# ducha-aiki/mods-light-zmq

Measured on AMD Instinct MI355X. Metric: image_pairs_per_sec_end_to_end, higher is better.
Workload: dtype f32

## Files before the change

include/mods_hip.h:

```cpp
#ifndef MODS_HIP_H
#define MODS_HIP_H

#include <stddef.h>
#include <stdint.h>

#ifdef __cplusplus
extern "C" {
#endif

#define MODS_OK 0
#define MODS_E_NODEVICE (-1)
#define MODS_E_ARG (-2)
#define MODS_E_CAPACITY (-3)
#define MODS_E_HIP (-4)

typedef struct mods_ctx mods_ctx;

typedef struct mods_hessaff_params {
  int numberOfScales;
  float initialSigma;
  float threshold;
  float edgeEigenValueRatio;
  int border;
  int maxIterations;
  float convergenceThreshold;
  int smmWindowSize;
  int doBaumberg;
  int mode;
  float relativeThreshold;
  int regionsNumber;
  float relativeRegionsNumber;
  int detectorType;
  int iiDoGMode;
  int sampleFromImage;
  double mserMaxArea;
  double mserMinMargin;
  int mserMinSize;
  int affBmbrgMethod;
} mods_hessaff_params;
enum { MODS_DET_FIXED_TH = 0, MODS_DET_RELATIVE_TH, MODS_DET_FIXED_REG_NUMBER, MODS_DET_RELATIVE_REG_NUMBER,
       MODS_DET_NOT_LESS_THAN_REGIONS };
enum { MODS_DET_HESSIAN = 0, MODS_DET_DOG = 1, MODS_DET_HARRIS = 2, MODS_DET_MSER = 3 };

typedef struct mods_affkey {
  double x, y, s, a11, a12, a21, a22, response;
  int sub_type;
  int octave, level, r0, c0;
  int pad;
} mods_affkey;

typedef struct mods_candidate {
  int octave, level, r0, c0, r, c;
  float x, y, s, pixelDistance, response;
  int type;
} mods_candidate;

typedef struct mods_region {
  double x, y, s, a11, a12, a21, a22, response;
  int sub_type;
  int id, parent;
  int pad;
  uint8_t desc[128];
} mods_region;

typedef struct mods_tentative {
  int q, t;
  int t_bad, t_2nd;
  float d1, d2, d2nd;
  float pad;
  double ratio;
} mods_tentative;

const char *mods_last_error(void);
int mods_device_count(void);
int mods_ctx_create(int device, int max_w, int max_h, int batch, mods_ctx **out);
int mods_ctx_create_ex(int device, int max_w, int max_h, int batch, int flags, mods_ctx **out);
void mods_ctx_destroy(mods_ctx *ctx);
int mods_ctx_sync(mods_ctx *ctx);
void *mods_ctx_stream(mods_ctx *ctx);

enum { MODS_STAGE_BLUR = 0, MODS_STAGE_RESPONSE, MODS_STAGE_RESIZE, MODS_STAGE_NMS, MODS_STAGE_LOCALIZE,
       MODS_STAGE_BAUMBERG, MODS_STAGE_SORT, MODS_STAGE_ORIENT, MODS_STAGE_DESCRIBE, MODS_STAGE_MATCH,
       MODS_STAGE_RANSAC_SCORE, MODS_STAGE_SYNTH,
       MODS_STAGE_BLUR_SMALL,
       MODS_STAGE_PYRAMID,
       MODS_STAGE_MATCH_NN1,
       MODS_STAGE_EXTRACT,
       MODS_STAGE_SIFT,
       MODS_STAGE_GUIDED,
       MODS_STAGE_MATCH_MUTUAL,
       MODS_STAGE_OVERLAP,
       MODS_STAGE_COUNT };
int mods_ctx_timing_enable(mods_ctx *ctx, int stage_mask);
int mods_ctx_graphs(mods_ctx *ctx, int on);
long mods_ctx_graph_replays(const mods_ctx *ctx);
long mods_ctx_u8_source_calls(const mods_ctx *ctx);
int mods_ctx_u8_kernels(mods_ctx *ctx, int mask);
int mods_ctx_pyramid_streams(mods_ctx *ctx, int n);
int mods_ctx_timing_read(mods_ctx *ctx, int stage, double *total_ms, int *launches, double *bytes);
int mods_ctx_timing_reset(mods_ctx *ctx);

int mods_detect_hessian_affine(mods_ctx *ctx, const float *img, int w, int h, int stride,
                               const mods_hessaff_params *par, mods_affkey *out, int max_out, int *n_out);
int mods_detect_hessian_affine_dev(mods_ctx *ctx, const float *img_dev, int n_img, int w, int h, int stride,
                                   const mods_hessaff_params *par, mods_affkey *out_host, int max_out,
                                   int *n_out_host);

int mods_pyramid_octaves(mods_ctx *ctx);
int mods_pyramid_dims(mods_ctx *ctx, int octave, int *w, int *h);
int mods_pyramid_plane(mods_ctx *ctx, int img, int octave, int level, int kind, float *dst_host);
int mods_pyramid_candidates(mods_ctx *ctx, int img, mods_candidate *out, int max_out, int *n_out);
int mods_pyramid_nms_hits(mods_ctx *ctx, int img, int *out4, int max_out, int *n_out);

int mods_gauss_blur(mods_ctx *ctx, const float *src, int w, int h, float sigma, float *dst);
int mods_hessian_response(mods_ctx *ctx, const float *src, int w, int h, float norm, float *dst);
int mods_resize_half(mods_ctx *ctx, const float *src, int w, int h, float *dst, int *dw, int *dh);

typedef struct mods_describe_params {
  double ori_mrSize;
  int ori_patchSize;
  int ori_maxAngles;
  double ori_threshold;
  double desc_mrSize;
  int desc_patchSize;
  int photoNorm;
  int rootSift;
  double maxBinValue;
  int ori_halfMode;
  int addUpRight;
  int halfDesc;
  int fastExtraction;
} mods_describe_params;

int mods_orient_describe(mods_ctx *ctx, const float *img, int w, int h, int stride, const mods_affkey *keys,
                         int n_keys, const mods_describe_params *par, mods_region *out, int max_out, int *n_out);

int mods_orient_describe_u8(mods_ctx *ctx, const unsigned char *img_u8, int w, int h, int stride, const mods_affkey *keys,
                            int n_keys, const mods_describe_params *par, mods_region *out, int max_out, int *n_out);

int mods_detect_describe_dev(mods_ctx *ctx, const float *img_dev, int n_img, int w, int h, int stride,
                             const mods_hessaff_params *det, const mods_describe_params *desc,
                             int *n_detected_host, int *n_regions_host);
int mods_detect_describe_dev_u8(mods_ctx *ctx, const unsigned char *img_u8_dev, int n_img, int w, int h, int stride,
                                const mods_hessaff_params *det, const mods_describe_params *desc,
                                int *n_detected_host, int *n_regions_host);
typedef int (*mods_descriptor_fn)(void *user, const float *patches, int n, int ps, float *out, size_t out_cap_floats, int *dim);
int mods_ctx_set_external_descriptor(mods_ctx *ctx, mods_descriptor_fn fn, void *user, double mrSize, int patchSize);
int mods_ctx_set_external_shape(mods_ctx *ctx, mods_descriptor_fn fn, void *user, double mrSize, int patchSize);
int mods_ctx_set_external_orientation(mods_ctx *ctx, mods_descriptor_fn fn, void *user, double mrSize, int patchSize);
typedef struct mods_net mods_net;
enum { MODS_NET_AFFNET = 0, MODS_NET_ORINET = 1, MODS_NET_HARDNET = 2 };
int  mods_net_create(int device, int kind, const float *const *tensors, const size_t *n_floats, int n_tensors, mods_net **out);
void mods_net_destroy(mods_net *net);
int  mods_net_dim(const mods_net *net);
int  mods_net_chunk(void);
int  mods_net_forward(mods_net *net, const float *patches_host, int n, int quantise_u8, float *out_host);
int  mods_net_forward_dev(mods_net *net, void *hip_stream, const float *patches_dev, int n, int quantise_u8, float *out_dev);
int  mods_ctx_set_builtin_shape(mods_ctx *ctx, mods_net *net, double mrSize, int quantise_u8);
int  mods_ctx_set_builtin_orientation(mods_ctx *ctx, mods_net *net, double mrSize, int quantise_u8);
int  mods_ctx_set_builtin_descriptor(mods_ctx *ctx, mods_net *net, double mrSize, int quantise_u8);
int  mods_test_net_stage(mods_net *net, int stage, const float *in_host, int n, int quantise_u8, float *out_host, int *guard_ok);
int mods_patches_fetch(mods_ctx *ctx, int img, int ps, float *out, int max_regions, int *n_out);
int mods_baumberg_stats_enable(mods_ctx *ctx, int on);
int mods_baumberg_stats(mods_ctx *ctx, int img, unsigned long long *keypoints, unsigned long long *iterations);
int mods_unoriented_count(mods_ctx *ctx, int img);
int mods_regions_fetch(mods_ctx *ctx, int img, mods_region *out, int max_out, int *n_out);

int mods_dominant_angle(mods_ctx *ctx, const float *patch, int ps, double th, float *angle, int *found);
int mods_selftest_fast_sqrt(mods_ctx *ctx, unsigned long long *out5);
int mods_sift_patch(mods_ctx *ctx, const float *patch, int ps, int rootsift, double maxBinValue, uint8_t *out128);

typedef struct mods_view_geom {
  int identity;
  int w_rot, h_rot;
  int w_new, h_new;
  int ksize_x, ksize_y, pad;
  double rotation, tilt, zoom;
  double sigma_x, sigma_y;
  double H[9];
  double warpRot[6], warpTilt[6];
// ... 142 lines not shown
  int n_tentatives, n_unique, n_inliers;
  int ransac_samples, ransac_lo, ransac_rejects;
  double H[9];
  double ms_detect_describe, ms_match, ms_duplicates, ms_ransac;
  int gt_true, gt_ransac_inliers, gt_true_of_ransac;
} mods_ladder_result;

int mods_view_schedule(const double *scale_set, int n_scales, const double *tilt_set, int n_tilts, double phi_base,
                       mods_view_par *prev, int *n_prev, int prev_cap, mods_view_par *out, int max_out);
int mods_imgrep_create(mods_ctx *ctx, int capacity, mods_imgrep **out);
void mods_imgrep_destroy(mods_imgrep *rep);
int mods_imgrep_clear(mods_imgrep *rep);
int mods_imgrep_count(const mods_imgrep *rep);
const mods_region *mods_imgrep_regions_dev(const mods_imgrep *rep);
int mods_imgrep_append_ctx(mods_imgrep *rep, mods_ctx *ctx, int img);
int mods_imgrep_append_ctx_half(mods_imgrep *rep, mods_ctx *ctx, int img);
int mods_imgrep_append_dev(mods_imgrep *rep, const mods_region *src_dev, int n);
int mods_imgrep_append_host(mods_imgrep *rep, const mods_region *src, int n);
int mods_imgrep_fetch(mods_imgrep *rep, int begin, int count, mods_region *out);
int mods_match_reps(mods_ctx *ctx, const mods_imgrep *q, int q_begin, int q_end, const mods_imgrep *t, double ratio,
                    double contradDist, int nn, mods_tentative *out, double *u6_out, double *laf_out, int max_out, int *n_out);
int mods_match_ladder_dev(mods_ctx *ctx, const float *img1_dev, int w1, int h1, const float *img2_dev, int w2, int h2,
                          const mods_ladder_step *steps, int n_steps, int min_matches, const mods_pair_params *par,
                          mods_imgrep *rep1, mods_imgrep *rep2, mods_ladder_result *res, double *matches_out, int max_matches);

int mods_match_ladder_dets_dev(mods_ctx *ctx, const float *img1_dev, int w1, int h1, const float *img2_dev, int w2, int h2,
                               const mods_ladder_step *steps, const mods_hessaff_params *dets, int n_steps, int n_det, int min_matches,
                               const struct mods_pair_params *par, mods_imgrep **reps1, mods_imgrep **reps2, mods_ladder_result *res,
                               double *matches_out, int max_matches);

typedef struct mods_ladder_group {
  int n_dets, dets[8];
  double fginn_ratio, fginn_ratio_half;
  double dist_threshold, dist_threshold_half;
} mods_ladder_group;
int mods_match_ladder_groups_dev(mods_ctx *ctx, const float *img1_dev, int w1, int h1, const float *img2_dev, int w2, int h2,
                                 const mods_ladder_step *steps, const mods_hessaff_params *dets, const mods_ladder_group *groups ,
                                 int group_pos, int n_steps, int n_det, int min_matches, const struct mods_pair_params *par,
                                 mods_imgrep **reps1, mods_imgrep **reps2, mods_ladder_result *res, double *matches_out, int max_matches);

typedef struct mods_multi mods_multi;
int mods_multi_create(const int *devices, int n, int w, int h, int rep_capacity, mods_multi **out);
void mods_multi_destroy(mods_multi *m);
int mods_multi_uses_rccl(const mods_multi *m);
mods_imgrep *mods_multi_bank(mods_multi *m, int image);
mods_imgrep *mods_multi_bank_det(mods_multi *m, int image, int det);
int mods_match_ladder_multi(mods_multi *m, const float *img1_host, int w1, int h1, const float *img2_host, int w2, int h2,
                            const mods_ladder_step *steps, int n_steps, int min_matches, const mods_pair_params *par,
                            mods_ladder_result *res, double *matches_out, int max_matches);
int mods_match_ladder_groups_multi(mods_multi *m, const float *img1_host, int w1, int h1, const float *img2_host, int w2, int h2,
                                   const mods_ladder_step *steps, const mods_hessaff_params *dets, const mods_ladder_group *groups ,
                                   int group_pos, int n_steps, int n_det, int min_matches, const struct mods_pair_params *par,
                                   mods_ladder_result *res, double *matches_out, int max_matches);
int mods_match_reps_any(mods_ctx *ctx, const mods_imgrep *q, int q_begin, int q_end, const mods_imgrep *t, double ratio, double contradDist,
                        int nn, double distance, mods_tentative *out, double *u6_out, double *laf_out, int max_out, int *n_out);
int mods_regions_half_copy_dev(mods_ctx *ctx, int img, mods_region *dst_dev, int n);
int mods_multi_assign(const double *areas, int n, int n_dev, int *owner);

int mods_match_verify_reps(mods_ctx *ctx, mods_imgrep *rep1, mods_imgrep *rep2, double fginn_ratio, const mods_pair_params *par,
                           mods_ladder_result *res, double *matches_out, int max_matches);
int mods_host_alloc(size_t bytes, void **out);
int mods_host_free(void *p);
int mods_dev_alloc(size_t bytes, void **out);
int mods_dev_free(void *p);
int mods_dev_upload(void *dst_dev, const void *src_host, size_t bytes);
int mods_dev_download(void *dst_host, const void *src_dev, size_t bytes);

typedef struct mods_clahe_params { double clip_limit; int tiles_x, tiles_y; } mods_clahe_params;
int mods_clahe_dev(mods_ctx *ctx, const unsigned char *src_dev, int n_img, int w, int h, int src_stride,
                   const mods_clahe_params *par, void *dst_dev, int dst_stride, int dst_f32);
int mods_clahe(mods_ctx *ctx, const unsigned char *src_host, int w, int h, const mods_clahe_params *par, unsigned char *dst_host);

typedef struct mods_pipeline mods_pipeline;
int mods_pipeline_create(int device, int w, int h, const mods_pair_params *par, int gpu_workers, int verify_workers,
                         mods_pipeline **out);
int mods_pipeline_create_ex(int device, int w, int h, const mods_pair_params *par, int gpu_workers, int verify_workers,
                            int pairs_per_batch, mods_pipeline **out);
int mods_pipeline_create_clahe(int device, int w, int h, const mods_pair_params *par, int gpu_workers, int verify_workers,
                               int pairs_per_batch, const mods_clahe_params *clahe, mods_pipeline **out);
int mods_pipeline_capacity(const mods_pipeline *p);
int mods_pipeline_timing_enable(mods_pipeline *p, int stage_mask);
int mods_pipeline_timing_read(mods_pipeline *p, int stage, double *total_ms, int *launches, double *bytes);
long mods_pipeline_u8_source_calls(mods_pipeline *p);
long mods_pipeline_graph_replays(mods_pipeline *p);
int mods_pipeline_cpu_seconds(mods_pipeline *p, double *gpu_workers_s, double *verify_workers_s, int reset);
int mods_pipeline_submit(mods_pipeline *p, const float *img_dev, long tag);
int mods_pipeline_submit_host(mods_pipeline *p, const float *img_host, long tag);
int mods_pipeline_submit_host_u8(mods_pipeline *p, const unsigned char *img_host, long tag);
int mods_pipeline_next(mods_pipeline *p, mods_pair_result *res, long *tag);
int mods_pipeline_next_matches(mods_pipeline *p, mods_pair_result *res, long *tag, double *matches_out, int max_matches);
void mods_pipeline_destroy(mods_pipeline *p);

typedef struct mods_guided_params {
  int model_type;
  double model[9];
  double radius;
  double ratio;
  double contradDist;
  int max_dist;
  int one_to_one;
} mods_guided_params;
int mods_match_guided(mods_ctx *ctx, const mods_region *q, int n_q, const mods_region *t, int n_t,
                      const mods_guided_params *par, mods_tentative *out, double *u6_out, double *laf_out,
                      int max_out, int *n_out);
int mods_match_guided_reps(mods_ctx *ctx, const mods_imgrep *q, const mods_imgrep *t,
                           const mods_guided_params *par, mods_tentative *out, double *u6_out, double *laf_out,
                           int max_out, int *n_out);

typedef struct mods_overlap_params {
  double H[9];
  double max_error;
  int oriented;
  int one_to_one;
  int w1, h1, w2, h2;
} mods_overlap_params;
typedef struct mods_overlap_match { int q, t; double E, dist, diff; } mods_overlap_match;
typedef struct mods_overlap_counts { int n_q_common, n_t_common, n_matches; double repeatability; } mods_overlap_counts;
int mods_match_overlap(mods_ctx *ctx, const mods_region *q, int n_q, const mods_region *t, int n_t,
                       const mods_overlap_params *par, mods_overlap_match *out, int max_out, int *n_out,
                       mods_overlap_counts *counts);
int mods_match_overlap_reps(mods_ctx *ctx, const mods_imgrep *q, const mods_imgrep *t,
                            const mods_overlap_params *par, mods_overlap_match *out, int max_out, int *n_out,
                            mods_overlap_counts *counts);
int mods_ctx_overlap_splits(mods_ctx *ctx, int splits);

int mods_ctx_match_mutual(mods_ctx *ctx, int mode);
int mods_match_mutual_counts(mods_ctx *ctx, int *n_forward, int *n_kept);
int mods_pipeline_match_mutual(mods_pipeline *p, int mode);

#ifdef __cplusplus
}
#endif
#endif
```

mods-light-zmq_amd/__init__.py:

```python
import ctypes as C
import os
import subprocess

import numpy as np

PKG_DIR = os.path.dirname(os.path.abspath(__file__))
LIB_PATH = os.environ.get("MODS_LIB") or os.path.join(PKG_DIR, "libmodsgpu.so")

MODS_OK = 0
STAGES = ["blur", "response", "resize", "nms", "localize", "baumberg", "sort", "orient", "describe", "match",
          "ransac_score", "synth", "blur_small", "pyramid", "match_nn1", "extract", "sift", "guided", "match_mutual",
          "overlap"]


class ModsError(RuntimeError):
    pass


class HessAffParams(C.Structure):
    _fields_ = [("numberOfScales", C.c_int), ("initialSigma", C.c_float), ("threshold", C.c_float),
                ("edgeEigenValueRatio", C.c_float), ("border", C.c_int), ("maxIterations", C.c_int),
                ("convergenceThreshold", C.c_float), ("smmWindowSize", C.c_int), ("doBaumberg", C.c_int),
                ("mode", C.c_int), ("relativeThreshold", C.c_float), ("regionsNumber", C.c_int),
                ("relativeRegionsNumber", C.c_float), ("detectorType", C.c_int), ("iiDoGMode", C.c_int),
# ... 295 lines not shown
        params = params or HessAffParams.default()
        counts = (C.c_int * n_img)()
        out = np.zeros((n_img, max_out), AFFKEY_DTYPE) if fetch else None
        _check(lib().mods_detect_hessian_affine_dev(self.h, C.c_void_p(dev_ptr), n_img, w, h, w, C.byref(params),
                                                    out.ctypes.data_as(C.c_void_p) if fetch else None, max_out, counts))
        if fetch:
            return [out[i, :counts[i]].copy() for i in range(n_img)]
        return list(counts)

    def pyramid_octaves(self):
        return lib().mods_pyramid_octaves(self.h)

    def pyramid_dims(self, o):
        w, h = C.c_int(), C.c_int()
        _check(lib().mods_pyramid_dims(self.h, o, C.byref(w), C.byref(h)))
        return w.value, h.value

    def pyramid_plane(self, img, o, level, kind):
        w, h = self.pyramid_dims(o)
        out = np.empty((h, w), np.float32)
        _check(lib().mods_pyramid_plane(self.h, img, o, level, kind, _fp(out)))
        return out

    def pyramid_candidates(self, img=0, max_out=1 << 20):
        out = np.zeros(max_out, CAND_DTYPE)
        n = C.c_int()
        _check(lib().mods_pyramid_candidates(self.h, img, out.ctypes.data_as(C.c_void_p), max_out, C.byref(n)))
        return out[:n.value].copy()

    def pyramid_nms_hits(self, img=0, max_out=1 << 22):
        n = C.c_int()
        rc = lib().mods_pyramid_nms_hits(self.h, img, None, 0, C.byref(n))
        if rc not in (MODS_OK, -3):
            _check(rc)
        out = np.full((min(max(n.value, 0), max_out), 4), -1, np.int32)
        _check(lib().mods_pyramid_nms_hits(self.h, img, out.ctypes.data_as(C.c_void_p), len(out), C.byref(n)))
        return out[:int(np.count_nonzero(out[:, 1] >= 0))].copy(), n.value
    def orient_describe(self, img, keys, params=None, max_out=None):
        params = params or DescribeParams.default()
        a = np.ascontiguousarray(img, np.float32)
        k = np.ascontiguousarray(keys)
        max_out = max_out or len(k) + 1
        out = np.zeros(max_out, REGION_DTYPE)
        n = C.c_int()
        _check(lib().mods_orient_describe(self.h, _fp(a), a.shape[1], a.shape[0], a.shape[1], k.ctypes.data_as(C.c_void_p),
                                          len(k), C.byref(params), out.ctypes.data_as(C.c_void_p), max_out, C.byref(n)))
        return out[:n.value].copy()

    def orient_describe_u8(self, img_u8, keys, params=None, max_out=None):
        params = params or DescribeParams.default()
        a = np.asarray(img_u8)
        if a.dtype != np.uint8 or a.ndim != 2:
            raise ValueError("orient_describe_u8 takes a 2-d uint8 array")
        if a.strides[1] != 1 or a.strides[0] < a.shape[1]:
            a = np.ascontiguousarray(a)
        k = np.ascontiguousarray(keys)
        max_out = max_out or len(k) + 1
        out = np.zeros(max_out, REGION_DTYPE)
        n = C.c_int()
        _check(lib().mods_orient_describe_u8(self.h, C.c_void_p(a.ctypes.data), a.shape[1], a.shape[0], a.strides[0],
                                             k.ctypes.data_as(C.c_void_p), len(k), C.byref(params), out.ctypes.data_as(C.c_void_p),
                                             max_out, C.byref(n)))
        return out[:n.value].copy()

    def regions_fetch_half(self, img=0, max_out=1 << 18):
        out = np.zeros(max_out, REGION_DTYPE)
        n = C.c_int()
        _check(lib().mods_regions_fetch_half(self.h, img, out.ctypes.data_as(C.c_void_p), max_out, C.byref(n)))
        return out[:n.value].copy()

    def detect_describe_dev(self, dev_ptr, n_img, w, h, det=None, desc=None):
        det = det or HessAffParams.default()
        desc = desc or DescribeParams.default()
        nd, nr = (C.c_int * n_img)(), (C.c_int * n_img)()
        _check(lib().mods_detect_describe_dev(self.h, C.c_void_p(dev_ptr), n_img, w, h, w, C.byref(det), C.byref(desc), nd, nr))
        return list(nd), list(nr)

    def u8_source_calls(self):
        lib().mods_ctx_u8_source_calls.restype = C.c_long
        return int(lib().mods_ctx_u8_source_calls(self.h))

    def set_u8_kernels(self, mask):
        _check(lib().mods_ctx_u8_kernels(self.h, int(mask)))

    def set_match_mutual(self, mode):
        _check(lib().mods_ctx_match_mutual(self.h, int(mode)))

    def match_mutual_counts(self):
        nf, nk = C.c_int(), C.c_int()
        _check(lib().mods_match_mutual_counts(self.h, C.byref(nf), C.byref(nk)))
        return nf.value, nk.value

    def detect_describe_dev_u8(self, dev_ptr, n_img, w, h, det=None, desc=None, stride=None):
        det = det or HessAffParams.default()
        desc = desc or DescribeParams.default()
        nd, nr = (C.c_int * n_img)(), (C.c_int * n_img)()
        _check(lib().mods_detect_describe_dev_u8(self.h, C.c_void_p(dev_ptr), n_img, w, h, w if stride is None else int(stride),
                                                 C.byref(det), C.byref(desc), nd, nr))
        return list(nd), list(nr)

    def regions_fetch(self, img, max_out=1 << 18):
        n = C.c_int()
        _check(lib().mods_regions_fetch(self.h, img, None, 0, C.byref(n)))
        out = np.zeros(max(n.value, 1), REGION_DTYPE)
        _check(lib().mods_regions_fetch(self.h, img, out.ctypes.data_as(C.c_void_p), len(out), C.byref(n)))
        return out[:n.value].copy()

    def set_external_descriptor(self, fn_ptr, user, mr_size=3.0 * np.sqrt(3.0), patch_size=32):
        _check(lib().mods_ctx_set_external_descriptor(self.h, C.c_void_p(fn_ptr), C.c_void_p(user), C.c_double(mr_size), patch_size))

    def set_external_shape(self, fn_ptr, user, mr_size=3.0 * np.sqrt(3.0), patch_size=32):
        _check(lib().mods_ctx_set_external_shape(self.h, C.c_void_p(fn_ptr), C.c_void_p(user), C.c_double(mr_size), patch_size))

    def set_external_orientation(self, fn_ptr, user, mr_size=3.0 * np.sqrt(3.0), patch_size=32):
        _check(lib().mods_ctx_set_external_orientation(self.h, C.c_void_p(fn_ptr), C.c_void_p(user), C.c_double(mr_size), patch_size))

    def set_builtin_shape(self, net, mr_size=3.0 * np.sqrt(3.0), quantise=True):
        _slot_check("shape", net)
        _check(lib().mods_ctx_set_builtin_shape(self.h, net.h if net is not None else None, C.c_double(mr_size), 1 if quantise else 0))
        self._nets = dict(getattr(self, "_nets", {}), shape=net)

    def set_builtin_orientation(self, net, mr_size=3.0 * np.sqrt(3.0), quantise=True):
        _slot_check("orientation", net)
        _check(lib().mods_ctx_set_builtin_orientation(self.h, net.h if net is not None else None, C.c_double(mr_size), 1 if quantise else 0))
        self._nets = dict(getattr(self, "_nets", {}), orientation=net)

    def set_builtin_descriptor(self, net, mr_size=3.0 * np.sqrt(3.0), quantise=True):
        _slot_check("descriptor", net)
        _check(lib().mods_ctx_set_builtin_descriptor(self.h, net.h if net is not None else None, C.c_double(mr_size), 1 if quantise else 0))
        self._nets = dict(getattr(self, "_nets", {}), descriptor=net)

    def patches_fetch(self, img, ps, max_regions=1 << 17):
        n = C.c_int()
        out = np.zeros((max_regions, ps, ps), np.float32) if max_regions <= 4096 else None
        if out is None:
            cnt = C.c_int()
            _check(lib().mods_regions_fetch(self.h, img, None, 0, C.byref(cnt)))
            out = np.zeros((max(cnt.value, 1), ps, ps), np.float32)
        _check(lib().mods_patches_fetch(self.h, img, ps, _fp(out), out.shape[0], C.byref(n)))
        return out[:n.value].copy()

    def regions_copy_dev(self, img, dst_ptr, n):
        _check(lib().mods_regions_copy_dev(self.h, img, C.c_void_p(dst_ptr), n))

    def dominant_angle(self, patch, th=float(np.float32(0.8))):
        a = np.ascontiguousarray(patch, np.float32)
        ang, found = C.c_float(), C.c_int()
        _check(lib().mods_dominant_angle(self.h, _fp(a), a.shape[0], C.c_double(th), C.byref(ang), C.byref(found)))
        return bool(found.value), ang.value

    def selftest_fast_sqrt(self):
        out = (C.c_ulonglong * 5)()
        _check(lib().mods_selftest_fast_sqrt(self.h, out))
        return tuple(int(v) for v in out)

    def sift_patch(self, patch, rootsift=True, max_bin=0.2):
        a = np.ascontiguousarray(patch, np.float32)
        out = np.zeros(128, np.uint8)
        _check(lib().mods_sift_patch(self.h, _fp(a), a.shape[0], int(rootsift), C.c_double(max_bin),
                                     out.ctypes.data_as(C.c_void_p)))
        return out

    def warp_affine(self, img, M, dw, dh, cval=128.0):
        a = np.ascontiguousarray(img, np.float32)
        Mc = np.ascontiguousarray(M, np.float64).ravel()
        out = np.empty((dh, dw), np.float32)
# ... 605 lines not shown
def multi_assign(areas, n_dev):
    a = np.ascontiguousarray(areas, np.float64)
    owner = np.zeros(len(a), np.int32)
    _check(lib().mods_multi_assign(a.ctypes.data_as(C.c_void_p), len(a), n_dev, owner.ctypes.data_as(C.c_void_p)))
    return owner


def match_verify_reps(ctx, rep1, rep2, fginn_ratio=0.8, params=None, max_matches=0):
    params = params or PairParams.default()
    res = LadderResult()
    m = np.zeros((max(max_matches, 1), 4), np.float64)
    _check(lib().mods_match_verify_reps(ctx.h, rep1.h, rep2.h, C.c_double(fginn_ratio), C.byref(params), C.byref(res),
                                        m.ctypes.data_as(C.c_void_p) if max_matches else None, max_matches))
    return res, m[:min(res.n_inliers, max_matches)]


class PairParams(C.Structure):
    _fields_ = [("det", HessAffParams), ("desc", DescribeParams), ("fginn_ratio", C.c_double),
                ("contradDist", C.c_double), ("nn", C.c_int), ("dup_before_ransac", C.c_int),
                ("dup_dist", C.c_double), ("dup_mode", C.c_int), ("ransac", RansacParams)]

    @staticmethod
    def default():
        return PairParams(HessAffParams.default(), DescribeParams.default(), 0.8, 10.0, 50, 1, 2.0, 1,
                          RansacParams.default())


class PairResult(C.Structure):
    _fields_ = [("n_detected", C.c_int * 2), ("n_described", C.c_int * 2), ("n_tentatives", C.c_int),
                ("n_unique", C.c_int), ("n_inliers", C.c_int), ("ransac_samples", C.c_int), ("ransac_lo", C.c_int),
                ("ransac_rejects", C.c_int), ("H", C.c_double * 9), ("ms_detect_describe", C.c_double),
                ("ms_match", C.c_double), ("ms_duplicates", C.c_double), ("ms_ransac", C.c_double)]


def match_pair_dev(ctx, dev_ptr, w, h, params=None, max_matches=0):
    params = params or PairParams.default()
    res = PairResult()
    m = np.zeros((max(max_matches, 1), 4), np.float64)
    _check(lib().mods_match_pair_dev(ctx.h, C.c_void_p(dev_ptr), w, h, w, C.byref(params), C.byref(res),
                                     m.ctypes.data_as(C.c_void_p) if max_matches else None, max_matches))
    return res, m[:min(res.n_inliers, max_matches)]


class PinnedBuffer:

    def __init__(self, shape, dtype):
        self.shape, self.dtype = tuple(shape), np.dtype(dtype)
        self.nbytes = int(np.prod(self.shape)) * self.dtype.itemsize
        self.ptr = C.c_void_p()
        _check(lib().mods_host_alloc(C.c_size_t(self.nbytes), C.byref(self.ptr)))
        buf = (C.c_char * self.nbytes).from_address(self.ptr.value)
        self.array = np.frombuffer(buf, dtype=self.dtype).reshape(self.shape)

    def close(self):
        if self.ptr:
            self.array = None
            lib().mods_host_free(self.ptr)
            self.ptr = C.c_void_p()


class Pipeline:

    def __init__(self, device, w, h, params=None, gpu_workers=1, verify_workers=1, pairs_per_batch=1, clahe=None, mutual=0):
        self.params = params or PairParams.default()
        self.h = C.c_void_p()
        if clahe is not None:
            self.clahe = clahe
            _check(lib().mods_pipeline_create_clahe(device, w, h, C.byref(self.params), gpu_workers, verify_workers, pairs_per_batch,
                                                    C.byref(self.clahe), C.byref(self.h)))
        else:
            _check(lib().mods_pipeline_create_ex(device, w, h, C.byref(self.params), gpu_workers, verify_workers, pairs_per_batch,
                                                 C.byref(self.h)))
        self.capacity = lib().mods_pipeline_capacity(self.h)
        if mutual:
            try:
                self.set_match_mutual(mutual)
            except ModsError:
                self.close()
                raise

    def set_match_mutual(self, mode):
        _check(lib().mods_pipeline_match_mutual(self.h, int(mode)))

    def submit(self, dev_ptr, tag=0):
        _check(lib().mods_pipeline_submit(self.h, C.c_void_p(dev_ptr), C.c_long(tag)))

    def submit_host(self, host_ptr, tag=0, u8=False):
        fn = lib().mods_pipeline_submit_host_u8 if u8 else lib().mods_pipeline_submit_host
        _check(fn(self.h, C.c_void_p(host_ptr), C.c_long(tag)))

    def next(self):
        res, tag = PairResult(), C.c_long()
        _check(lib().mods_pipeline_next(self.h, C.byref(res), C.byref(tag)))
        return res, tag.value

    def next_matches(self, max_matches=1 << 16):
        res, tag = PairResult(), C.c_long()
        m = np.zeros((max_matches, 4), np.float64)
        _check(lib().mods_pipeline_next_matches(self.h, C.byref(res), C.byref(tag), m.ctypes.data_as(C.c_void_p), max_matches))
        return res, tag.value, m[:min(res.n_inliers, max_matches)]

    def timing_enable(self, stages):
        mask = 0
        for s in stages:
            mask |= 1 << STAGES.index(s)
        _check(lib().mods_pipeline_timing_enable(self.h, mask))

    def timing_read(self, stage):
        ms, n, by = C.c_double(), C.c_int(), C.c_double()
        _check(lib().mods_pipeline_timing_read(self.h, STAGES.index(stage), C.byref(ms), C.byref(n), C.byref(by)))
        return ms.value, n.value, by.value

    def graph_replays(self):
        lib().mods_pipeline_graph_replays.restype = C.c_long
        return int(lib().mods_pipeline_graph_replays(self.h))

    def u8_source_calls(self):
        lib().mods_pipeline_u8_source_calls.restype = C.c_long
        return int(lib().mods_pipeline_u8_source_calls(self.h))

    def cpu_seconds(self, reset=False):
        g, v = C.c_double(), C.c_double()
        _check(lib().mods_pipeline_cpu_seconds(self.h, C.byref(g), C.byref(v), 1 if reset else 0))
        return g.value, v.value

    def close(self):
        if self.h:
            lib().mods_pipeline_destroy(self.h)
            self.h = C.c_void_p()

    def __del__(self):
        try:
            self.close()
        except Exception:
            pass
```

mods-light-zmq_amd/csrc/capi.hip:

```cpp
#include "common.hpp"
#include "detmath.hpp"
#include "ransac_host.hpp"
#include "f_laf.hpp"
#include "../../include/mods_degensac.h"
#include <cstdarg>
#include <memory>
#include <algorithm>
#include <cmath>
#include <mutex>
#include <vector>
#include <time.h>
#include <sys/prctl.h>

namespace mods {

static thread_local char g_err[512] = "";

void set_error(const char *fmt, ...) {
  va_list ap;
  va_start(ap, fmt);
  vsnprintf(g_err, sizeof(g_err), fmt, ap);
  va_end(ap);
}

// ... 301 lines not shown
int mods_pyramid_plane(mods_ctx *c, int img, int o, int level, int kind, float *dst) {
  if (o < 0 || o >= c->pyr.n_oct || level < 0 || level >= c->pyr.n_levels || img < 0 || img >= c->last_n_img) return MODS_E_ARG;
  const OctaveDev &oc = c->pyr.oct[o];
  const float *p = (kind ? oc.resp[level] : oc.blur[level]) + (size_t)oc.w * oc.h * img;
  MODS_HIP_CHECK(mods::stream_wait(c->stream));
  MODS_HIP_CHECK(mods::copy_wait(c->stream, dst, p, sizeof(float) * (size_t)oc.w * oc.h, hipMemcpyDeviceToHost));
  return MODS_OK;
}
int mods_pyramid_candidates(mods_ctx *c, int img, mods_candidate *out, int max_out, int *n_out) {
  MODS_HIP_CHECK(mods::stream_wait(c->stream));
  int count = 0;
  MODS_HIP_CHECK(mods::copy_wait(c->stream, &count, c->cand_count + img, sizeof(int), hipMemcpyDeviceToHost));
  int n = std::min(count, c->max_cand);
  std::vector<CandDev> v(n);
  MODS_HIP_CHECK(mods::copy_wait(c->stream, v.data(), c->cand + (size_t)img * c->max_cand, sizeof(CandDev) * n, hipMemcpyDeviceToHost));
  int m = 0;
  for (auto &cd : v) {
    if (!(cd.state == 2 || cd.state == 3 || cd.state == 4)) continue;
    if (m < max_out) {
      mods_candidate &o = out[m];
      o.octave = cd.octave; o.level = cd.level; o.r0 = cd.r0; o.c0 = cd.c0; o.r = cd.r; o.c = cd.c;
      o.x = cd.x; o.y = cd.y; o.s = cd.s; o.pixelDistance = cd.pixelDistance; o.response = cd.response; o.type = cd.type;
    }
    m++;
  }
  *n_out = m;
  return m > max_out ? MODS_E_CAPACITY : MODS_OK;
}
int mods_pyramid_nms_hits(mods_ctx *c, int img, int *out4, int max_out, int *n_out) {
  if (!c || !n_out || img < 0 || img >= c->batch || (max_out > 0 && !out4)) { set_error("pyramid_nms_hits: bad argument"); return MODS_E_ARG; }
  MODS_HIP_CHECK(hipSetDevice(c->device));
  MODS_HIP_CHECK(mods::stream_wait(c->stream));
  int count = 0;
  MODS_HIP_CHECK(mods::copy_wait(c->stream, &count, c->cand_count + img, sizeof(int), hipMemcpyDeviceToHost));
  *n_out = count;
  const int n = std::max(0, std::min(count, c->max_cand));
  if (n > max_out) { set_error("NMS hit output overflow: %d > %d", n, max_out); return MODS_E_CAPACITY; }
  std::vector<CandDev> v(n);
  MODS_HIP_CHECK(mods::copy_wait(c->stream, v.data(), c->cand + (size_t)img * c->max_cand, sizeof(CandDev) * n, hipMemcpyDeviceToHost));
  for (int i = 0; i < n; i++) {
    out4[4 * i] = v[i].octave; out4[4 * i + 1] = v[i].level; out4[4 * i + 2] = v[i].r0; out4[4 * i + 3] = v[i].c0;
  }
  return MODS_OK;
}

static int check_desc_err(mods_ctx *c) {
  int e = 0;
  MODS_HIP_CHECK(hipMemcpyAsync(&e, c->desc_err_dev, sizeof(int), hipMemcpyDeviceToHost, c->stream));
  MODS_HIP_CHECK(mods::stream_wait(c->stream));
  if (e) {
    MODS_HIP_CHECK(hipMemsetAsync(c->desc_err_dev, 0, sizeof(int), c->stream));
    set_error("measurement region larger than the descriptor scratch (P2 > 3*max(w,h) or > 4096 blur taps)");
    return MODS_E_CAPACITY;
  }
  return MODS_OK;
}

static int dd_enqueue(mods_ctx *c, const float *img_dev, int n_img, int w, int h, int stride, const mods_hessaff_params *det,
                      const mods_describe_params *desc) {
  int rc;
  if ((rc = detect_any(c, img_dev, n_img, w, h, stride, det, 1.0, 1.0))) return rc;
  const float *planes = img_dev;
  if (stride != w) planes = c->tmp_dev;
  if ((rc = describe_run(c, planes, n_img, w, h, desc))) return rc;
  int *hc = c->host_counts;
  MODS_HIP_CHECK(hipMemcpyAsync(hc, c->cand_count, sizeof(int) * 3 * c->batch, hipMemcpyDeviceToHost, c->stream));
  MODS_HIP_CHECK(hipMemcpyAsync(hc + 3 * c->batch, c->region_count, sizeof(int) * c->batch, hipMemcpyDeviceToHost, c->stream));
  MODS_HIP_CHECK(hipMemcpyAsync(hc + 4 * c->batch, c->inside_count, sizeof(int) * n_img, hipMemcpyDeviceToHost, c->stream));
  MODS_HIP_CHECK(hipMemcpyAsync(hc + 5 * c->batch, c->desc_err_dev, sizeof(int), hipMemcpyDeviceToHost, c->stream));
  return MODS_OK;
}

static unsigned long long fnv1a(const void *p, size_t n, unsigned long long h) {
  const unsigned char *b = (const unsigned char *)p;
  for (size_t i = 0; i < n; i++) { h ^= b[i]; h *= 1099511628211ull; }
  return h;
}

static int dd_run(mods_ctx *c, const float *img_dev, int n_img, int w, int h, int stride, const mods_hessaff_params *det,
                  const mods_describe_params *desc) {
  const bool can = c->dd_graphs && c->timing_mask == 0 && !mods::has_hooks(c) && !mods::has_nets(c) && det->detectorType != MODS_DET_MSER;
  if (!can) { mods::dev_state_changed(c); return dd_enqueue(c, img_dev, n_img, w, h, stride, det, desc); }
  mods_ctx::DdKey key;
  key.img = img_dev; key.img_u8 = c->img_u8_dev; key.n_img = n_img; key.w = w; key.h = h; key.stride = stride;
  key.par_hash = fnv1a(desc, sizeof(*desc), fnv1a(det, sizeof(*det), 1469598103934665603ull)) ^ (unsigned long long)c->pyr_streams;
  key.epoch = c->dev_state_epoch;
  if (c->dd_stale) { dd_graph_drop(c); c->dd_linear.clear(); c->dd_stale = false; }
  const bool repeat = key == c->dd_prev;
  c->dd_prev = key;
  if (!repeat) return dd_enqueue(c, img_dev, n_img, w, h, stride, det, desc);
  for (auto &e : c->dd_cache)
    if (e.first == key) {
      MODS_HIP_CHECK(hipGraphLaunch(e.second, c->stream));
      c->dd_replays++;
      return MODS_OK;
    }
  for (const auto &k2 : c->dd_linear)
    if (k2 == key) return dd_enqueue(c, img_dev, n_img, w, h, stride, det, desc);
  hipStream_t s = c->stream;
  if (hipStreamBeginCapture(s, hipStreamCaptureModeThreadLocal) != hipSuccess) {
    (void)hipGetLastError();
    c->dd_graphs = false;
    return dd_enqueue(c, img_dev, n_img, w, h, stride, det, desc);
  }
  const int rc = dd_enqueue(c, img_dev, n_img, w, h, stride, det, desc);
  hipGraph_t g = nullptr;
  const hipError_t e_end = hipStreamEndCapture(s, &g);
  hipGraphExec_t ex = nullptr;
  if (rc == MODS_OK && e_end == hipSuccess && g && !c->pyr_forked) {
    (void)hipGraphDestroy(g);
    if (c->dd_linear.size() >= 16) c->dd_linear.erase(c->dd_linear.begin());
    c->dd_linear.push_back(key);
    return dd_enqueue(c, img_dev, n_img, w, h, stride, det, desc);
  }
  if (rc == MODS_OK && e_end == hipSuccess && g && hipGraphInstantiate(&ex, g, nullptr, nullptr, 0) == hipSuccess) {
    (void)hipGraphDestroy(g);
    if (c->dd_cache.size() >= 8) { (void)hipGraphExecDestroy(c->dd_cache.front().second); c->dd_cache.erase(c->dd_cache.begin()); }
    c->dd_cache.emplace_back(key, ex);
    MODS_HIP_CHECK(hipGraphLaunch(ex, c->stream));
    c->dd_replays++;
    return MODS_OK;
  }
  if (g) (void)hipGraphDestroy(g);
  (void)hipGetLastError();
  c->pyr_side = false;
  c->dd_graphs = false;
  c->omap_dirty = true;
  return dd_enqueue(c, img_dev, n_img, w, h, stride, det, desc);
}

int mods_ctx_graphs(mods_ctx *c, int on) {
  if (!c) return MODS_E_ARG;
  c->dd_graphs = on != 0;
  if (!on) { dd_graph_drop(c); c->dd_linear.clear(); }
  mods::dev_state_changed(c);
  return MODS_OK;
}
long mods_ctx_graph_replays(const mods_ctx *c) { return c ? c->dd_replays : 0; }
long mods_ctx_u8_source_calls(const mods_ctx *c) { return c ? c->u8_source_calls : 0; }
int mods_ctx_u8_kernels(mods_ctx *c, int mask) {
  if (!c || mask > 15) { set_error("u8_kernels: bad argument"); return MODS_E_ARG; }
  c->u8_kernels = mask < 0 ? -1 : mask;
  mods::dev_state_changed(c);
  return MODS_OK;
}

static int dd_call(mods_ctx *c, const float *img_dev, int n_img, int w, int h, int stride, const mods_hessaff_params *det,
                   const mods_describe_params *desc, int *n_detected_host, int *n_regions_host) {
  int rc;
  if ((rc = dd_run(c, img_dev, n_img, w, h, stride, det, desc))) return rc;
  int *hc = c->host_counts;
  MODS_HIP_CHECK(mods::stream_wait(c->stream));
  for (int b = 0; b < n_img; b++) {
    if (hc[b] > c->max_cand) { set_error("NMS hit list overflow: %d > %d", hc[b], c->max_cand); return MODS_E_CAPACITY; }
    if (n_detected_host) n_detected_host[b] = hc[2 * c->batch + b];
    if (hc[3 * c->batch + b] > std::min(c->max_cand, 1 << 17)) { set_error("region list overflow: %d", hc[3 * c->batch + b]); return MODS_E_CAPACITY; }
    if (n_regions_host) n_regions_host[b] = hc[3 * c->batch + b];
  }
  c->last_region_counts.assign(hc + 3 * c->batch, hc + 3 * c->batch + n_img);
  c->last_inside_counts.assign(hc + 4 * c->batch, hc + 4 * c->batch + n_img);
  if (hc[5 * c->batch]) {
    MODS_HIP_CHECK(hipMemsetAsync(c->desc_err_dev, 0, sizeof(int), c->stream));
    set_error("measurement region larger than the descriptor scratch (P2 > 3*max(w,h) or > 4096 blur taps)");
    return MODS_E_CAPACITY;
  }
  return MODS_OK;
}

int mods_detect_describe_dev(mods_ctx *c, const float *img_dev, int n_img, int w, int h, int stride,
                             const mods_hessaff_params *det, const mods_describe_params *desc, int *n_detected_host,
                             int *n_regions_host) {
  if (!c || !img_dev || !det || !desc) { set_error("detect_describe: null argument"); return MODS_E_ARG; }
  if (w <= 0 || h <= 0 || (size_t)w * h > (size_t)c->max_w * c->max_h) { set_error("detect_describe: image larger than the context"); return MODS_E_ARG; }
  if (n_img < 1 || n_img > c->batch) { set_error("detect_describe: %d images, context batch %d", n_img, c->batch); return MODS_E_ARG; }
  if (stride < w) { set_error("detect_describe: stride %d < width %d", stride, w); return MODS_E_ARG; }
  MODS_HIP_CHECK(hipSetDevice(c->device));
  c->img_u8_dev = nullptr;
  return dd_call(c, img_dev, n_img, w, h, stride, det, desc, n_detected_host, n_regions_host);
}

int mods_detect_describe_dev_u8(mods_ctx *c, const unsigned char *img_u8_dev, int n_img, int w, int h, int stride,
                                const mods_hessaff_params *det, const mods_describe_params *desc, int *n_detected_host,
                                int *n_regions_host) {
  if (!c || !img_u8_dev || !det || !desc) { set_error("detect_describe_u8: null argument"); return MODS_E_ARG; }
  if (w <= 0 || h <= 0 || (size_t)w * h > (size_t)c->max_w * c->max_h) { set_error("detect_describe_u8: image larger than the context"); return MODS_E_ARG; }
  if (n_img < 1 || n_img > c->batch) { set_error("detect_describe_u8: %d images, context batch %d", n_img, c->batch); return MODS_E_ARG; }
  if (stride < w) { set_error("detect_describe_u8: stride %d < width %d", stride, w); return MODS_E_ARG; }
  MODS_HIP_CHECK(hipSetDevice(c->device));
  int rc;
  if ((rc = mods::u8_to_f32_launch(c, img_u8_dev, n_img, w, h, stride, c->input_dev))) return rc;
  c->img_u8_dev = (stride == w && det->detectorType != MODS_DET_MSER) ? img_u8_dev : nullptr;
  if (c->img_u8_dev) c->u8_source_calls++;
  rc = dd_call(c, c->input_dev, n_img, w, h, w, det, desc, n_detected_host, n_regions_host);
  c->img_u8_dev = nullptr;
  return rc;
}

int mods_ctx_set_external_descriptor(mods_ctx *c, mods_descriptor_fn fn, void *user, double mrSize, int patchSize) {
  if (!c) return MODS_E_ARG;
  c->ext_fn = fn; c->ext_user = user; c->ext_mr = mrSize; c->ext_ps = patchSize;
  c->ext_net = nullptr;
  return MODS_OK;
}

int mods_ctx_set_external_shape(mods_ctx *c, mods_descriptor_fn fn, void *user, double mrSize, int patchSize) {
  if (!c) return MODS_E_ARG;
  if (fn && (patchSize < 8 || patchSize > 63)) { set_error("external shape: patch size %d unsupported", patchSize); return MODS_E_ARG; }
  c->shape_fn = fn; c->shape_user = user; c->shape_mr = mrSize; c->shape_ps = patchSize;
  c->shape_net = nullptr;
  return MODS_OK;
}

int mods_ctx_set_external_orientation(mods_ctx *c, mods_descriptor_fn fn, void *user, double mrSize, int patchSize) {
  if (!c) return MODS_E_ARG;
  if (fn && (patchSize < 8 || patchSize > 63)) { set_error("external orientation: patch size %d unsupported", patchSize); return MODS_E_ARG; }
  c->ori_fn = fn; c->ori_user = user; c->ori_mr = mrSize; c->ori_ps = patchSize;
  c->ori_net = nullptr;
  return MODS_OK;
}
int mods_patches_fetch(mods_ctx *c, int img, int ps, float *out, int max_regions, int *n_out) {
  if (!c || !out || !n_out || img < 0 || img >= c->batch || !c->desc_scratch) { set_error("patches_fetch: nothing described"); return MODS_E_ARG; }
  const int reg_cap = std::min(c->max_cand, 1 << 17);
  MODS_HIP_CHECK(hipSetDevice(c->device));
  MODS_HIP_CHECK(mods::stream_wait(c->stream));
  int n = 0;
  MODS_HIP_CHECK(mods::copy_wait(c->stream, &n, c->region_count + img, sizeof(int), hipMemcpyDeviceToHost));
  if (n > reg_cap) n = reg_cap;
  if (n > max_regions) { set_error("patch output overflow: %d > %d", n, max_regions); return MODS_E_CAPACITY; }
  MODS_HIP_CHECK(mods::copy_wait(c->stream, out, c->desc_scratch + (size_t)img * reg_cap * ps * ps, sizeof(float) * (size_t)n * ps * ps, hipMemcpyDeviceToHost));
  *n_out = n;
  return MODS_OK;
}

int mods_baumberg_stats_enable(mods_ctx *c, int on) {
  if (!c) return MODS_E_ARG;
  MODS_HIP_CHECK(hipSetDevice(c->device));
  MODS_HIP_CHECK(mods::stream_wait(c->stream));
  c->baum_stats_dev.release();
  mods::dev_pool_reallocated(c);
  if (on) {
    const size_t n = 2 * 64 * (size_t)c->batch;
    MODS_HIP_CHECK(c->baum_stats_dev.reserve(n));
    MODS_HIP_CHECK(mods::fill_wait(c->stream, c->baum_stats_dev, 0, sizeof(unsigned long long) * n));
  }
  return MODS_OK;
}
int mods_baumberg_stats(mods_ctx *c, int img, unsigned long long *keypoints, unsigned long long *iterations) {
  if (!c || img < 0 || img >= c->batch || !c->baum_stats_dev) return MODS_E_ARG;
  MODS_HIP_CHECK(hipSetDevice(c->device));
  MODS_HIP_CHECK(mods::stream_wait(c->stream));
  unsigned long long v[2 * 64], kp = 0, it = 0;
  MODS_HIP_CHECK(mods::copy_wait(c->stream, v, c->baum_stats_dev + 2 * 64 * (size_t)img, sizeof(v), hipMemcpyDeviceToHost));
  for (int q = 0; q < 64; q++) { kp += v[2 * q]; it += v[2 * q + 1]; }
  if (keypoints) *keypoints = kp;
  if (iterations) *iterations = it;
  return MODS_OK;
}

int mods_unoriented_count(mods_ctx *c, int img) {
  if (!c || img < 0 || img >= (int)c->last_inside_counts.size()) return 0;
  return c->last_inside_counts[img];
}

int mods_regions_fetch(mods_ctx *c, int img, mods_region *out, int max_out, int *n_out) {
  if (!c || img < 0 || img >= c->batch || !n_out) return MODS_E_ARG;
  MODS_HIP_CHECK(hipSetDevice(c->device));
  MODS_HIP_CHECK(mods::stream_wait(c->stream));
  int n = 0;
  MODS_HIP_CHECK(mods::copy_wait(c->stream, &n, c->region_count + img, sizeof(int), hipMemcpyDeviceToHost));
  *n_out = n;
  if (out) {
    if (n > max_out) { set_error("region output overflow: %d > %d", n, max_out); return MODS_E_CAPACITY; }
    MODS_HIP_CHECK(mods::copy_wait(c->stream, out, c->regions_dev + (size_t)img * c->max_cand, sizeof(mods_region) * n, hipMemcpyDeviceToHost));
  }
  return MODS_OK;
}

int mods_regions_fetch_half(mods_ctx *c, int img, mods_region *out, int max_out, int *n_out) {
  if (!c || img < 0 || img >= c->batch || !n_out) return MODS_E_ARG;
  if (!c->have_half || !c->regions_half_dev) { set_error("no HalfRootSIFT descriptors: the last describe call did not ask for them"); return MODS_E_ARG; }
  MODS_HIP_CHECK(hipSetDevice(c->device));
  MODS_HIP_CHECK(mods::stream_wait(c->stream));
  int n = 0;
  MODS_HIP_CHECK(mods::copy_wait(c->stream, &n, c->region_count + img, sizeof(int), hipMemcpyDeviceToHost));
  *n_out = n;
  if (out) {
    if (n > max_out) { set_error("region output overflow: %d > %d", n, max_out); return MODS_E_CAPACITY; }
    MODS_HIP_CHECK(mods::copy_wait(c->stream, out, c->regions_half_dev + (size_t)img * c->max_cand, sizeof(mods_region) * n, hipMemcpyDeviceToHost));
  }
  return MODS_OK;
}
const mods_region *mods_regions_half_dev(mods_ctx *c, int img) {
  return (c && c->have_half && c->regions_half_dev) ? c->regions_half_dev + (size_t)img * c->max_cand : nullptr;
}

int mods_orient_describe(mods_ctx *c, const float *img, int w, int h, int stride, const mods_affkey *keys, int n_keys,
                         const mods_describe_params *par, mods_region *out, int max_out, int *n_out) {
  if (!c || !img || !par || !n_out || (n_keys > 0 && !keys)) { set_error("orient_describe: null argument"); return MODS_E_ARG; }
  if ((size_t)w * h > (size_t)c->max_w * c->max_h) { set_error("image larger than the context"); return MODS_E_ARG; }
  if (n_keys > c->max_cand) { set_error("too many keypoints for the context: %d > %d", n_keys, c->max_cand); return MODS_E_CAPACITY; }
  MODS_HIP_CHECK(hipSetDevice(c->device));
  MODS_HIP_CHECK(hipMemcpy2DAsync(c->input_dev, sizeof(float) * w, img, sizeof(float) * stride, sizeof(float) * w, h,
                                  hipMemcpyHostToDevice, c->stream));
  MODS_HIP_CHECK(hipMemcpyAsync(c->keys_dev, keys, sizeof(mods_affkey) * n_keys, hipMemcpyHostToDevice, c->stream));
  MODS_HIP_CHECK(hipMemcpyAsync(c->cand_count + 2 * c->batch, &n_keys, sizeof(int), hipMemcpyHostToDevice, c->stream));
  MODS_HIP_CHECK(mods::stream_wait(c->stream));
  int rc = describe_run(c, c->input_dev, 1, w, h, par);
  if (rc) return rc;
  if ((rc = mods_regions_fetch(c, 0, out, max_out, n_out))) return rc;
  return check_desc_err(c);
}

int mods_orient_describe_u8(mods_ctx *c, const unsigned char *img_u8, int w, int h, int stride, const mods_affkey *keys, int n_keys,
                            const mods_describe_params *par, mods_region *out, int max_out, int *n_out) {
  if (!img_u8 || !par || !n_out || (n_keys > 0 && !keys)) { set_error("orient_describe_u8: null argument"); return MODS_E_ARG; }
  if (w < 1 || h < 1) { set_error("orient_describe_u8: image size %d x %d", w, h); return MODS_E_ARG; }
  if (stride < w) { set_error("orient_describe_u8: stride %d < width %d", stride, w); return MODS_E_ARG; }
  if (n_keys < 0) { set_error("orient_describe_u8: %d keypoints", n_keys); return MODS_E_ARG; }
  if (!c) { set_error("orient_describe_u8: null context"); return MODS_E_ARG; }
  if ((size_t)w * h > (size_t)c->max_w * c->max_h) { set_error("orient_describe_u8: image %d x %d larger than the context", w, h); return MODS_E_ARG; }
  if (n_keys > c->max_cand) { set_error("orient_describe_u8: too many keypoints for the context: %d > %d", n_keys, c->max_cand); return MODS_E_ARG; }
  MODS_HIP_CHECK(hipSetDevice(c->device));
  int rc;
  if ((rc = mods::u8_stage_ensure(c))) return rc;
  MODS_HIP_CHECK(hipMemcpy2DAsync(c->u8_stage_dev, w, img_u8, stride, w, h, hipMemcpyHostToDevice, c->stream));
  MODS_HIP_CHECK(hipMemcpyAsync(c->keys_dev, keys, sizeof(mods_affkey) * n_keys, hipMemcpyHostToDevice, c->stream));
  MODS_HIP_CHECK(hipMemcpyAsync(c->cand_count + 2 * c->batch, &n_keys, sizeof(int), hipMemcpyHostToDevice, c->stream));
  MODS_HIP_CHECK(mods::stream_wait(c->stream));
  if ((rc = mods::u8_to_f32_launch(c, c->u8_stage_dev, 1, w, h, w, c->input_dev))) return rc;
  c->img_u8_dev = c->u8_stage_dev;
  c->u8_source_calls++;
  rc = describe_run(c, c->input_dev, 1, w, h, par);
  c->img_u8_dev = nullptr;
  if (rc) return rc;
  if ((rc = mods_regions_fetch(c, 0, out, max_out, n_out))) return rc;
  return check_desc_err(c);
}

int mods_dominant_angle(mods_ctx *c, const float *patch, int ps, double th, float *angle, int *found) {
  mods_describe_params dp = {5.1962, ps, 1, th, 5.1962, c->desc_ps ? c->desc_ps : 41, 1, 1, 0.2};
  MODS_HIP_CHECK(hipSetDevice(c->device));
  int rc = describe_configure(c, &dp);
  if (rc) return rc;
  MODS_HIP_CHECK(hipMemcpyAsync(c->input_dev, patch, sizeof(float) * ps * ps, hipMemcpyHostToDevice, c->stream));
  if ((rc = launch_dominant_angle_test(c, c->input_dev, ps, th, c->tmp_dev))) return rc;
  float res[2];
  MODS_HIP_CHECK(hipMemcpyAsync(res, c->tmp_dev, sizeof(res), hipMemcpyDeviceToHost, c->stream));
  MODS_HIP_CHECK(mods::stream_wait(c->stream));
  *found = res[0] != 0.f;
  *angle = res[1];
  return MODS_OK;
}

int mods_selftest_fast_sqrt(mods_ctx *c, unsigned long long *out5) {
  if (!c || !out5) { set_error("selftest: null argument"); return MODS_E_ARG; }
  MODS_HIP_CHECK(hipSetDevice(c->device));
  return launch_fast_sqrt_selftest(c, out5);
}

int mods_sift_patch(mods_ctx *c, const float *patch, int ps, int rootsift, double maxBinValue, uint8_t *out128) {
  mods_describe_params dp = {5.1962, c->desc_ori_ps ? c->desc_ori_ps : 32, 1, 0.8, 5.1962, ps, 1, rootsift, maxBinValue};
  MODS_HIP_CHECK(hipSetDevice(c->device));
  int rc = describe_configure(c, &dp);
  if (rc) return rc;
  MODS_HIP_CHECK(hipMemcpyAsync(c->input_dev, patch, sizeof(float) * ps * ps, hipMemcpyHostToDevice, c->stream));
  if ((rc = launch_sift_patch_test(c, c->input_dev, ps, rootsift, maxBinValue, (uint8_t *)c->tmp_dev.get()))) return rc;
  MODS_HIP_CHECK(hipMemcpyAsync(out128, c->tmp_dev, 128, hipMemcpyDeviceToHost, c->stream));
  MODS_HIP_CHECK(mods::stream_wait(c->stream));
  return MODS_OK;
}

int mods_match_copy_out(mods_ctx *c, int n, mods_tentative *tent, double *u6, double *laf) {
  if (n <= 0) return MODS_OK;
  static thread_local std::vector<char> stage;
  stage.resize(tent_bytes((size_t)n));
  MODS_HIP_CHECK(hipMemcpyAsync(stage.data(), c->m_tent, stage.size(), hipMemcpyDeviceToHost, c->stream));
  MODS_HIP_CHECK(mods::stream_wait(c->stream));
  tent_unpack(stage.data(), (size_t)n, tent, u6, laf);
  return MODS_OK;
}

int mods_match_fetch_internal(mods_ctx *c, mods_tentative *out, double *u6_out, double *laf_out, int max_out, int *n_out) {
  MODS_HIP_CHECK(mods::stream_wait(c->stream));
  const int n = read_slot(c->m_count, count_slot());
  *n_out = n;
  if (n > max_out) { set_error("tentative output overflow: %d > %d", n, max_out); return MODS_E_CAPACITY; }
  return mods_match_copy_out(c, n, out, u6_out, laf_out);
}

static int match_upload(mods_ctx *c, const mods_region *q, int n_q, const mods_region *t, int n_t, const int *n_out) {
  if (!c || !n_out || (n_q > 0 && !q) || (n_t > 0 && !t)) { set_error("match: null argument"); return MODS_E_ARG; }
  MODS_HIP_CHECK(hipSetDevice(c->device));
  int rc = match_ensure_buffers(c);
  if (rc) return rc;
  if (n_q > c->max_cand || n_t > c->max_cand) { set_error("match: list larger than the context capacity"); return MODS_E_CAPACITY; }
  MODS_HIP_CHECK(hipMemcpyAsync(c->m_regs, q, sizeof(mods_region) * n_q, hipMemcpyHostToDevice, c->stream));
  MODS_HIP_CHECK(hipMemcpyAsync(c->m_regs + c->max_cand, t, sizeof(mods_region) * n_t, hipMemcpyHostToDevice, c->stream));
  return MODS_OK;
}

int mods_match_fginn(mods_ctx *c, const mods_region *q, int n_q, const mods_region *t, int n_t, double ratio,
                     double contradDist, int nn, mods_tentative *out, double *u6_out, double *laf_out, int max_out, int *n_out) {
  int rc = match_upload(c, q, n_q, t, n_t, n_out);
  if (rc || (rc = match_run(c, c->m_regs, n_q, c->m_regs + c->max_cand, n_t, ratio, contradDist, nn))) return rc;
  return mods_match_fetch_internal(c, out, u6_out, laf_out, max_out, n_out);
}

int mods_match_distance(mods_ctx *c, const mods_region *q, int n_q, const mods_region *t, int n_t, double threshold,
                        mods_tentative *out, double *u6_out, double *laf_out, int max_out, int *n_out) {
  int rc = match_upload(c, q, n_q, t, n_t, n_out);
  if (rc || (rc = match_run_distance(c, c->m_regs, n_q, c->m_regs + c->max_cand, n_t, threshold))) return rc;
  return mods_match_fetch_internal(c, out, u6_out, laf_out, max_out, n_out);
}

int mods_match_dev(mods_ctx *c, int img_q, int img_t, double ratio, double contradDist, int nn, mods_tentative *out,
                   double *u6_out, double *laf_out, int max_out, int *n_out) {
// ... 379 lines not shown
```

mods-light-zmq_amd/csrc/common.hpp:

```cpp
#pragma once
#include <hip/hip_runtime.h>
#include <atomic>
#include <chrono>
#include <cmath>
#include <cstdint>
#include <cstdio>
#include <cstring>
#include <string>
#include <vector>
#include "../../include/mods_hip.h"
#include "buffer.hpp"

namespace mods {

void set_error(const char *fmt, ...);

#define MODS_HIP_CHECK(expr)                                                              \
  do {                                                                                    \
    hipError_t _e = (expr);                                                               \
    if (_e != hipSuccess) {                                                               \
      mods::set_error("%s failed: %s (%s:%d)", #expr, hipGetErrorString(_e), __FILE__, __LINE__); \
      return MODS_E_HIP;                                                                  \
    }                                                                                     \
  } while (0)
// ... 87 lines not shown
}

struct TentList {
  std::vector<mods_tentative> tent;
  std::vector<double> u6, laf;
  size_t size() const { return tent.size(); }
  bool empty() const { return tent.empty(); }
  void clear() { tent.clear(); u6.clear(); laf.clear(); }
  void resize(size_t n) { tent.resize(n); u6.resize(n * 6); laf.resize(n * 14); }
  void truncate(size_t n) { if (n < size()) resize(n); }
  void append(const TentList &o) {
    tent.insert(tent.end(), o.tent.begin(), o.tent.end());
    u6.insert(u6.end(), o.u6.begin(), o.u6.end());
    laf.insert(laf.end(), o.laf.begin(), o.laf.end());
  }
  void unpack_from(const char *packed, size_t n) { resize(n); tent_unpack(packed, n, tent.data(), u6.data(), laf.data()); }
  void pack_into(char *packed) const { tent_pack(packed, size(), tent.data(), u6.data(), laf.data()); }
  void copy_matches(int n, double *matches_out, int max_matches) const {
    if (!matches_out) return;
    for (int m = 0; m < n && m < max_matches && (size_t)m < size(); m++) {
      const double *p = &u6[(size_t)m * 6];
      matches_out[4 * m] = p[0]; matches_out[4 * m + 1] = p[1]; matches_out[4 * m + 2] = p[3]; matches_out[4 * m + 3] = p[4];
    }
  }
};

constexpr int kCountSlots = 64;
constexpr int kCountInts = 3 * kCountSlots;
constexpr int kLastSearch = -1;
constexpr int count_slot(int pair = kLastSearch) { return 1 + pair; }
constexpr int kept_slot(int pair = kLastSearch) { return kCountSlots + 1 + pair; }
constexpr int status_slot(int pair = kLastSearch) { return 2 * kCountSlots + 1 + pair; }
inline int read_slot(const int *counts, int slot) { return ((const volatile int *)counts)[slot]; }

struct MserState;

}

struct mods_ctx {
  mods_ctx() = default;
  ~mods_ctx();
  int device = 0;
  int n_cu = 256;
  int max_w = 0, max_h = 0, batch = 1;
  hipStream_t stream = nullptr;
  hipEvent_t pyr_scope_begin = nullptr;
  hipStream_t stream2 = nullptr;
  hipEvent_t ev_fork = nullptr, ev_join = nullptr;
  bool pyr_side = false;
  int pyr_side_first = 0;
  int pyr_streams = 2;
  mods::PyramidDev pyr;
  mods::Buf<mods::PyramidDev> pyr_dev;
  mods::PyramidDev pyr_dev_image;
  bool pyr_dev_valid = false;
  mods::Buf<float> plane_pool;
  mods::Buf<unsigned int> omap_pool;
  bool omap_dirty = true;
  mods::Buf<float> input_dev;
  mods::Buf<float> tmp_dev;
  mods::Buf<float> alt_taps_dev;
  int alt_ntap[mods::kMaxLevels] = {0};
  float alt_sigma[mods::kMaxLevels] = {0};
  mods::Buf<float> alt_planes;
  mods::Buf<float> view_dev;
  mods::Buf<float> gauss_taps_dev;
  float taps_sigma[16] = {0};
  float taps_host[16][2 * mods::kMaxBlurRadius + 1] = {{0}};
  int taps_host_n[16] = {0};
  mods::Buf<float> smm_mask_dev;
  mods::Buf<unsigned long long> baum_stats_dev;
  int smm_mask_size = 0;
  int max_cand = 0;
  mods::Buf<mods::CandDev> cand;
  mods::Buf<int> cand_count;
  mods::Buf<mods_affkey> keys_dev;
  mods::Buf<unsigned long long> sort_keys;
  mods::Buf<int> sort_idx;
  mods::Buf<int> rank_dev;
  mods::Buf<unsigned long long> nms_mask;
  mods::PinnedBuf<int> host_counts;
  mods::Buf<unsigned char> u8_stage_dev;
  const unsigned char *img_u8_dev = nullptr;
  int u8_kernels = -1;
  long u8_source_calls = 0;
  mods::Buf<unsigned char> clahe_lut;
  bool clahe_on = false;
  mods_clahe_params clahe_par = {0.0, 0, 0};
  mods::PinnedBuf<char> pin_arena;
  mods_hessaff_params par;
  int reg_number_eff = -1;
  int last_w = 0, last_h = 0, last_n_img = 0;
  const float *last_img_dev = nullptr; int last_stride = 0;
  mods::Buf<float> desc_tables_dev;
  mods::Buf<int> desc_err_dev;
  int desc_ori_ps = 0, desc_ps = 0;
  mods::Buf<char> ori_dev;
  mods::Buf<char> ori_multi_dev;
  mods::Buf<mods_region> regions_dev;
  mods::Buf<mods_region> regions_half_dev;
  bool have_half = false;
  mods::Buf<int> region_count;
  mods::Buf<int> inside_count;
  std::vector<int> last_inside_counts;
  mods::Buf<float> desc_scratch;
  int blur_table_ps = 0;
  mods::Buf<float> blur_table_dev;
  mods_descriptor_fn ext_fn = nullptr;
  void *ext_user = nullptr;
  double ext_mr = 0;
  int ext_ps = 0;
  mods_descriptor_fn shape_fn = nullptr, ori_fn = nullptr;
  void *shape_user = nullptr, *ori_user = nullptr;
  double shape_mr = 0, ori_mr = 0;
  int shape_ps = 0, ori_ps = 0;
  mods_net *shape_net = nullptr, *ori_net = nullptr, *ext_net = nullptr;
  int shape_q8 = 0, ori_q8 = 0, ext_q8 = 0;
  mods::Buf<float> net_out_dev;
  std::vector<int> last_region_counts;
  mods::Buf<int8_t> m_desc;
  mods::Buf<int> m_c;
  mods::Buf<double2> m_xy;
  mods::Buf<unsigned long long> m_u64;
  mods::Buf<int> m_int;
  mods::Buf<char> m_mid;
  mods::Buf<char> m_p2;
  size_t m_best2_cap = 0;
  int m_sets = 0;
  mods::Buf<char> m_tent;
  mods::PinnedBuf<int> m_count;
  mods_tentative *m_tent_out = nullptr; int *m_count_out = nullptr;
  mods::Buf<char> m_tent_batch;
  mods::Buf<mods_region> m_regs;
  mods::Buf<char> dd_buf; int dd_jobs = 0;
  mods::Buf<char> m_tent2;
  mods::TentList h_list;
  std::vector<unsigned char> h_mask;
  mods::Buf<double4> g_rec;
  mods::Buf<unsigned char> g_desc;
  mods::Buf<unsigned long long> g_key;
  mods::Buf<int> g_int;
  mods::Buf<char> g_tent;
  mods::Buf<mods_region> g_regs;
  mods::PinnedBuf<int> g_count;
  mods::Buf<double> o_rec;
  mods::Buf<unsigned long long> o_key;
  mods::Buf<int> o_int;
  mods::Buf<mods_overlap_match> o_out;
  mods::Buf<mods_region> o_regs;
  mods::PinnedBuf<int> o_count;
  int o_splits = 0;
  int mutual_mode = 0;
  bool mu_last_checked = false;
  mods::Buf<int4> mu_cand;
  mods::PinnedBuf<int> mu_count;
  mods::MserState *mser = nullptr;
  std::vector<mods_ctx *> helpers;
  std::atomic<bool> helpers_failed{false};
  std::vector<mods::Buf<mods_region>> helper_stage;
  int timing_mask = 0;
  bool dd_graphs = false;
  struct DdKey { const float *img = nullptr; const unsigned char *img_u8 = nullptr;
                 int n_img = 0, w = 0, h = 0, stride = 0; unsigned long long par_hash = 0, epoch = ~0ull;
                 bool operator==(const DdKey &o) const { return img == o.img && img_u8 == o.img_u8 && n_img == o.n_img && w == o.w && h == o.h && stride == o.stride && par_hash == o.par_hash && epoch == o.epoch; } };
  unsigned long long dev_state_epoch = 0;
  std::vector<std::pair<DdKey, hipGraphExec_t>> dd_cache;
  bool dd_stale = false;
  DdKey dd_prev;
  std::vector<DdKey> dd_linear;
  bool pyr_forked = false;
  long dd_replays = 0;
  mods::StageTimer timers[MODS_STAGE_COUNT];
};

namespace mods {

constexpr int kTabOriMask = 0, kTabDescMask = 4096, kTabVoteMask = 8192, kTabSift = 12288;

inline void dev_state_changed(mods_ctx *c) { c->dev_state_epoch++; }
inline void dev_pool_reallocated(mods_ctx *c) { c->dev_state_epoch++; c->dd_stale = true; }

template <class B> inline hipError_t reserve_scratch(mods_ctx *c, B &b, size_t need, size_t alloc_elems, bool *moved = nullptr) {
  if (need <= b.capacity()) return hipSuccess;
  if (b.get()) { const hipError_t e = stream_wait(c->stream); if (e != hipSuccess) return e; }
  return b.reserve(need, alloc_elems, moved);
}
template <class B> inline hipError_t reserve_pool(mods_ctx *c, B &b, size_t need, size_t alloc_elems) {
  bool moved = false;
  const hipError_t e = reserve_scratch(c, b, need, alloc_elems, &moved);
  if (moved) dev_pool_reallocated(c);
  return e;
}
struct StageScope {
  mods_ctx *ctx; int stage; hipEvent_t e0 = nullptr, e1 = nullptr; bool on;
  StageScope(mods_ctx *c, int s, double bytes = 0);
  ~StageScope();
};

int pyramid_configure(mods_ctx *ctx, int w, int h, int n_img, const mods_hessaff_params *par);
int pyramid_build(mods_ctx *ctx, const float *img_dev, int stride);
int pyramid_join_side(mods_ctx *ctx);
int launch_gauss_blur(mods_ctx *ctx, const float *src, float *dst, int w, int h, int n_img, float sigma);
int launch_hessian_response(mods_ctx *ctx, const float *src, float *dst, int w, int h, int n_img, float norm);
int launch_resize_half(mods_ctx *ctx, const float *src, float *dst, int w, int h, int dw, int dh, int n_img);
void resize_half_dims(int w, int h, int *dw, int *dh);
int gauss_ksize(float sigma);
void gauss_kernel_host(int n, double sigma, float *out);
void gauss_mask_host(int size, float *out);
void circular_gauss_mask_host(int size, float sigma, float *out);

int clahe_reserve(mods_ctx *ctx, int n_img, const mods_clahe_params *par);
int clahe_launch(mods_ctx *ctx, const unsigned char *src, int n_img, int w, int h, int src_stride, const mods_clahe_params *par,
                 void *dst, int dst_stride, int dst_f32);

int detect_run(mods_ctx *ctx);

int detect_any(mods_ctx *ctx, const float *img_dev, int n_img, int w, int h, int stride, const mods_hessaff_params *par, double tilt,
               double zoom);
void mser_release(mods_ctx *ctx);

int match_run(mods_ctx *ctx, const mods_region *q_dev, int n_q, const mods_region *t_dev, int n_t, double ratio,
              double contradDist, int nn);
int match_run_distance(mods_ctx *ctx, const mods_region *q_dev, int n_q, const mods_region *t_dev, int n_t, double threshold);
int match_ensure_buffers(mods_ctx *ctx, int n_sets = 1);
int match_run_group(mods_ctx *ctx, int n_jobs, const mods_region *const *q_dev, const int *n_q, const mods_region *const *t_dev, const int *n_t,
                    mods_tentative *const *tent_out, int *const *count_out, double ratio, double contradDist, int nn);

constexpr int DUP_MAX_JOBS = 64;
struct DupJob { const char *src; char *dst; const int *n_src; int *n_dst; int *status; };
int dup_filter_dev(mods_ctx *c, const DupJob *jobs, int n_jobs, int grid_n, double r, int mode);
int dup_filter_reserve(mods_ctx *c, int n_jobs);
static_assert(DUP_MAX_JOBS <= kCountSlots, "every job of the duplicate filter has its slots in m_count");
int launch_fast_sqrt_selftest(mods_ctx *ctx, unsigned long long *out5_host);
int launch_blur_table(mods_ctx *ctx, int ps);
bool ransac_profile_on();
int ransac_profile_mode();

int describe_run(mods_ctx *ctx, const float *img_dev, int n_img, int w, int h, const mods_describe_params *par);
int u8_to_f32_launch(mods_ctx *c, const unsigned char *src, int n_img, int w, int h, int stride, float *dst);
int u8_stage_ensure(mods_ctx *c);
int describe_run_view(mods_ctx *ctx, const float *img_dev, int n_img, int w, int h, const mods_describe_params *par, const double *H,
                      int orig_w, int orig_h, mods_region *det_copy_dev);
int describe_configure(mods_ctx *ctx, const mods_describe_params *par);
int launch_dominant_angle_test(mods_ctx *ctx, const float *patch_dev, int ps, double th, float *out_dev);
int launch_sift_patch_test(mods_ctx *ctx, const float *patch_dev, int ps, int root, double max_bin, uint8_t *out_dev);

inline bool has_hooks(const mods_ctx *c) { return c->ext_fn || c->shape_fn || c->ori_fn; }
inline bool has_nets(const mods_ctx *c) { return c->ext_net || c->shape_net || c->ori_net; }
int net_run_to_host(mods_ctx *ctx, mods_net *net, const float *patches_dev, int n, int quantise_u8, float *out_host);

int pair_gpu_stage(mods_ctx *c, const float *img_dev, int w, int h, int stride, const mods_pair_params *par, mods_pair_result *res,
                   TentList *list);
int pairs_gpu_stage(mods_ctx *c, const void *const *img, const int *kinds, int n_pairs, int w, int h, const mods_pair_params *par,
                    mods_pair_result *const *res, TentList *const *lists);
int pair_verify_stage(int device, const mods_pair_params *par, mods_pair_result *res, TentList *list, double *matches_out,
                      int max_matches, int w, int h);

}

extern "C" {
int mods_match_copy_out(mods_ctx *c, int n, mods_tentative *tent, double *u6, double *laf);
int mods_match_fetch_internal(mods_ctx *c, mods_tentative *out, double *u6_out, double *laf_out, int max_out, int *n_out);
int mods_ransac_warmup(int device, int len);
int mods_ctx_warmup(mods_ctx *c, int n_img, int w, int h, const mods_pair_params *par);
}
```

mods-light-zmq_amd/csrc/describe.hip:

```cpp
#include "describe_common.hpp"
#include "detmath.hpp"
#include "device_util.hpp"

namespace mods {

struct OriOut { double a11, a12, a21, a22; int alive; int pad; };

__device__ unsigned char g_ori_bin[2048];
__global__ __launch_bounds__(256) void ori_bin_table_kernel() {
  const float PIf = 3.14159265358979323846f;
  const int bins = 36;
  const int e = blockIdx.x * 256 + threadIdx.x;
  const float ori = atan2_lut_case(e >> 8, g_atan_lut[e & 255]);
  g_ori_bin[e] = (unsigned char)(int)(bins * (ori / PIf + 1.0f) / 2.0f);
}

__device__ __forceinline__ float peak_angle(const float *s_hist, int b) {
  const int bins = 36;
  const float PIf = 3.14159265358979323846f;
  const int a = b == 0 ? bins - 1 : b - 1, c = b == bins - 1 ? 0 : b + 1;
  const float ha = s_hist[a], hb = s_hist[b], hc = s_hist[c];
  const float pp = (ha - hc) / (ha - 2.0f * hb + hc) / 2.0f;
  return 2.0f * PIf * (b + 0.5f + pp) / bins - PIf;
}
// ... 612 lines not shown
      if (ctx->ori_net) {
        if ((rc = net_run_to_host(ctx, ctx->ori_net, ctx->desc_scratch + (size_t)b * k.reg_cap * kNetPS * kNetPS, n, ctx->ori_q8, out.data()))) return rc;
      } else {
        int dim = 0;
        const int frc = ctx->ori_fn(ctx->ori_user, patches[b].data(), n, ctx->ori_ps, out.data(), out.size(), &dim);
        if (frc || dim != 2) { set_error("external orientation function failed (rc %d, %d values per patch; 2 expected)", frc, dim); return MODS_E_ARG; }
      }
      for (int i = 0; i < n; i++) {
        mods_region r = regs[b][i];
        const double angle = atan2f(out[2 * i], out[2 * i + 1]);
        double ci, si;
        det_sincos(angle, &si, &ci);
        const double a11 = r.a11, a12 = r.a12, a21 = r.a21, a22 = r.a22;
        r.a11 = a11 * ci - a12 * si;
        r.a12 = a11 * si + a12 * ci;
        r.a21 = a21 * ci - a22 * si;
        r.a22 = a21 * si + a22 * ci;
        const int box = (int)(k.ks * r.s);
        bool alive = true;
        if (k.view) {
          const double rx = (k.Hinv[0] * r.x + k.Hinv[1] * r.y + k.Hinv[2]);
          const double ry = (k.Hinv[3] * r.x + k.Hinv[4] * r.y + k.Hinv[5]);
          const double r11 = (k.Hinv[0] * r.a11 + k.Hinv[1] * r.a21), r12 = (k.Hinv[0] * r.a12 + k.Hinv[1] * r.a22);
          const double r21 = (k.Hinv[3] * r.a11 + k.Hinv[4] * r.a21), r22 = (k.Hinv[3] * r.a12 + k.Hinv[4] * r.a22);
          if (!((rx < k.ow) && (ry < k.oh) && (rx > 0) && (ry > 0))) alive = false;
          else if (check_borders(k.ow, k.oh, (float)rx, (float)ry, (float)r11, (float)r12, (float)r21, (float)r22, box, box)) alive = false;
        } else if (check_borders(k.w, k.h, (float)r.x, (float)r.y, (float)r.a11, (float)r.a12, (float)r.a21, (float)r.a22, box, box)) alive = false;
        if (!alive) continue;
        r.parent = r.id; r.id = (int)kept.size();
        kept.push_back(r);
      }
    }
    counts[b] = (int)kept.size();
    if (counts[b] > k.reg_cap) counts[b] = k.reg_cap;
    if (counts[b]) MODS_HIP_CHECK(mods::copy_wait(ctx->stream, ctx->regions_dev + (size_t)b * ctx->max_cand, kept.data(), sizeof(mods_region) * counts[b], hipMemcpyHostToDevice));
  }
  MODS_HIP_CHECK(mods::copy_wait(ctx->stream, ctx->region_count, counts.data(), sizeof(int) * n_img, hipMemcpyHostToDevice));
  MODS_HIP_CHECK(mods::copy_wait(ctx->stream, ctx->inside_count, inside.data(), sizeof(int) * n_img, hipMemcpyHostToDevice));
  return MODS_OK;
}

static void invert3_cv(const double *S, double *t) {
  double d = S[0] * (S[4] * S[8] - S[5] * S[7]) - S[1] * (S[3] * S[8] - S[5] * S[6]) + S[2] * (S[3] * S[7] - S[4] * S[6]);
  if (d == 0.) { for (int i = 0; i < 9; i++) t[i] = 0; return; }
  d = 1. / d;
  t[0] = (S[4] * S[8] - S[5] * S[7]) * d; t[1] = (S[2] * S[7] - S[1] * S[8]) * d; t[2] = (S[1] * S[5] - S[2] * S[4]) * d;
  t[3] = (S[5] * S[6] - S[3] * S[8]) * d; t[4] = (S[0] * S[8] - S[2] * S[6]) * d; t[5] = (S[2] * S[3] - S[0] * S[5]) * d;
  t[6] = (S[3] * S[7] - S[4] * S[6]) * d; t[7] = (S[1] * S[6] - S[0] * S[7]) * d; t[8] = (S[0] * S[4] - S[1] * S[3]) * d;
}

int describe_run_view(mods_ctx *ctx, const float *img_dev, int n_img, int w, int h, const mods_describe_params *par, const double *H,
                      int orig_w, int orig_h, mods_region *det_copy_dev) {
  int rc = describe_configure(ctx, par);
  if (rc) return rc;
  DescConst k;
  k.view = 0; k.ow = w; k.oh = h;
  for (int i = 0; i < 6; i++) k.Hinv[i] = (i == 0 || i == 4) ? 1.0 : 0.0;
  if (H) {
    const bool eye = (std::fabs(H[0] - 1.0) + std::fabs(H[1]) + std::fabs(H[2]) + std::fabs(H[3]) + std::fabs(H[4] - 1.0) + std::fabs(H[5]) +
                      std::fabs(H[6]) + std::fabs(H[7]) + std::fabs(H[8] - 1.0) < 0.01);
    k.ow = orig_w; k.oh = orig_h;
    if (!eye) {
      double Hi[9];
      invert3_cv(H, Hi);
      k.view = 1;
      for (int i = 0; i < 6; i++) k.Hinv[i] = Hi[i];
    } else if (orig_w != w || orig_h != h) k.view = 1;
  }
  k.w = w; k.h = h; k.max_cand = ctx->max_cand; k.max_reg = ctx->max_cand;
  k.reg_cap = std::min(ctx->max_cand, 1 << 17);
  k.ks = 2 * 3.0 * sqrt(3.0);
  k.ori_ps = par->ori_patchSize;
  k.ori_i2p = double(2 * int(par->ori_mrSize) + 1) / (double)par->ori_patchSize;
  k.max_angles = par->ori_maxAngles;
  k.ori_cap = std::max(1, std::min(par->ori_maxAngles, 18));
  k.ori_th = par->ori_threshold;
  k.ori_half = par->ori_halfMode; k.half_desc = 0; k.add_upright = par->addUpRight;
  k.desc_mr = par->desc_mrSize; k.desc_ps = par->desc_patchSize; k.photo = par->photoNorm; k.root = par->rootSift;
  k.max_bin = par->maxBinValue;
  k.patch_rule = par->fastExtraction ? 2 : 0;
  const bool external = ctx->ext_fn != nullptr || ctx->ext_net != nullptr;
  const bool hooks = external || ctx->shape_fn || ctx->shape_net || ctx->ori_fn || ctx->ori_net;
  const unsigned char *img_u8 = (!H && !hooks) ? ctx->img_u8_dev : nullptr;
  if (external && par->fastExtraction) { set_error("FastPatchExtraction with an external descriptor is not supported"); return MODS_E_ARG; }
  if (external) { k.desc_mr = ctx->ext_mr; k.desc_ps = ctx->ext_ps; k.photo = 0; k.patch_rule = 1; }
  int *key_count = ctx->cand_count + 2 * ctx->batch;
  const float *orimask = ctx->desc_tables_dev + kTabVoteMask, *dmask = ctx->desc_tables_dev + kTabDescMask;
  const SiftTab *tab = (const SiftTab *)(ctx->desc_tables_dev + kTabSift);
  if ((ctx->shape_fn || ctx->shape_net) && ctx->par.detectorType == MODS_DET_HESSIAN && (rc = external_shape(ctx, img_dev, n_img, k, key_count, dmask, tab))) return rc;
  if (ctx->ori_fn || ctx->ori_net) {
    if ((rc = external_orientation(ctx, img_dev, n_img, k, key_count, dmask, tab))) return rc;
  } else {
    StageScope ts(ctx, MODS_STAGE_ORIENT);
    const size_t lds = orient_lds_bytes(k.ori_ps);
    hipLaunchKernelGGL(ori_bin_table_kernel, dim3(8), dim3(256), 0, ctx->stream);
    if (k.ori_cap > 1) {
      const size_t need = sizeof(OriOut) * (size_t)k.ori_cap * ctx->max_cand * ctx->batch;
      MODS_HIP_CHECK(mods::reserve_pool(ctx, ctx->ori_multi_dev, need, need));
    }
    if (img_u8 && kernel_from_u8(ctx, U8K_ORIENT))
      hipLaunchKernelGGL(orient_kernel<unsigned char>, dim3(8192, n_img), dim3(64), lds, ctx->stream, img_u8, k, ctx->keys_dev, key_count,
                         orimask, (OriOut *)ctx->ori_dev.get(), (OriOut *)ctx->ori_multi_dev.get());
    else
      hipLaunchKernelGGL(orient_kernel<float>, dim3(8192, n_img), dim3(64), lds, ctx->stream, img_dev, k, ctx->keys_dev, key_count,
                         orimask, (OriOut *)ctx->ori_dev.get(), (OriOut *)ctx->ori_multi_dev.get());
    if (k.ori_cap > 1)
      hipLaunchKernelGGL(compact_regions_multi_kernel, dim3(1, n_img), dim3(1024), 0, ctx->stream, k, ctx->keys_dev, key_count,
                         (const OriOut *)ctx->ori_dev.get(), (const OriOut *)ctx->ori_multi_dev.get(), ctx->regions_dev, ctx->region_count, ctx->inside_count);
    else
      hipLaunchKernelGGL(compact_regions_kernel, dim3((ctx->max_cand + 1023) / 1024, n_img), dim3(1024), 0, ctx->stream, k, ctx->keys_dev, key_count,
                         (const OriOut *)ctx->ori_dev.get(), ctx->regions_dev, ctx->region_count, ctx->inside_count);
    MODS_HIP_CHECK(hipGetLastError());
  }
  rc = launch_extract_and_sift(ctx, img_dev, n_img, k, dmask, tab, !external, img_u8);
  if (rc) return rc;
  ctx->have_half = false;
  if (par->halfDesc && !external) {
    if ((rc = launch_half_sift(ctx, n_img, k, dmask, tab))) return rc;
    ctx->have_half = true;
  }
  if (external && (rc = external_describe(ctx, n_img, k))) return rc;
  if (det_copy_dev)
    MODS_HIP_CHECK(hipMemcpyAsync(det_copy_dev, ctx->regions_dev, sizeof(mods_region) * (size_t)ctx->max_cand, hipMemcpyDeviceToDevice, ctx->stream));
  if (k.view) {
    hipLaunchKernelGGL(reproject_regions_kernel, dim3(256, n_img), dim3(256), 0, ctx->stream, k, ctx->regions_dev, ctx->region_count);
    if (ctx->have_half)
      hipLaunchKernelGGL(reproject_regions_kernel, dim3(256, n_img), dim3(256), 0, ctx->stream, k, ctx->regions_half_dev, ctx->region_count);
    MODS_HIP_CHECK(hipGetLastError());
  }
  return MODS_OK;
}

int launch_dominant_angle_test(mods_ctx *ctx, const float *patch_dev, int ps, double th, float *out_dev) {
  const size_t lds = orient_lds_bytes(ps);
  hipLaunchKernelGGL(ori_bin_table_kernel, dim3(8), dim3(256), 0, ctx->stream);
  hipLaunchKernelGGL(dominant_angle_test_kernel, dim3(1), dim3(64), lds, ctx->stream, patch_dev, ps, th,
                     ctx->desc_tables_dev + kTabVoteMask, out_dev);
  MODS_HIP_CHECK(hipGetLastError());
  return MODS_OK;
}

}
```

mods-light-zmq_amd/csrc/describe_common.hpp:

```cpp
#pragma once
#include "common.hpp"

namespace mods {

struct DescConst {
  int w, h;
  int max_cand, max_reg;
  int reg_cap;
  double ks;
  int ori_ps;
  double ori_i2p;
  int max_angles;
  int ori_cap;
  double ori_th;
  int ori_half;
  int add_upright;
  int half_desc;
  double desc_mr;
  int desc_ps;
  int photo, root;
  double max_bin;
  int p2_lo, p2_hi;
  size_t scratch_stride;
  int tap_cap;
  int patch_rule;
  int view;
  int ow, oh;
  double Hinv[6];
};

struct SiftTab {
  int bin0[64], bin1[64];
  float w0[64], w1[64];
};

#ifndef ORIENT_FROM_U8
#define ORIENT_FROM_U8 0
#endif
#ifndef EXTRACT_SMALL_FROM_U8
#define EXTRACT_SMALL_FROM_U8 1
#endif
#ifndef BIG_FUSED_FROM_U8
#define BIG_FUSED_FROM_U8 1
#endif
#ifndef BIG_SAMPLE_FROM_U8
#define BIG_SAMPLE_FROM_U8 0
#endif
enum { U8K_ORIENT = 1, U8K_EXTRACT_SMALL = 2, U8K_BIG_FUSED = 4, U8K_BIG_SAMPLE = 8 };
constexpr int kU8KernelsDefault = (ORIENT_FROM_U8 ? U8K_ORIENT : 0) | (EXTRACT_SMALL_FROM_U8 ? U8K_EXTRACT_SMALL : 0) |
                                  (BIG_FUSED_FROM_U8 ? U8K_BIG_FUSED : 0) | (BIG_SAMPLE_FROM_U8 ? U8K_BIG_SAMPLE : 0);
inline bool kernel_from_u8(const mods_ctx *ctx, int kernel) { return ((ctx->u8_kernels < 0 ? kU8KernelsDefault : ctx->u8_kernels) & kernel) != 0; }

int launch_extract_and_sift(mods_ctx *ctx, const float *img_dev, int n_img, DescConst k, const float *dmask, const SiftTab *tab,
                            bool run_sift = true, const unsigned char *img_u8 = nullptr);
int launch_half_sift(mods_ctx *ctx, int n_img, DescConst k, const float *dmask, const SiftTab *tab);
int launch_sift_patch_test(mods_ctx *ctx, const float *patch_dev, int ps, int root, double max_bin, uint8_t *out_dev);

}
```

mods-light-zmq_amd/csrc/device_util.hpp:

```cpp
#pragma once
#include <hip/hip_runtime.h>
#include "atan_lut_data.h"

namespace mods {

__host__ __device__ __forceinline__ bool check_borders(int img_w, int img_h, float ofsx, float ofsy, float a11, float a12,
                                              float a21, float a22, int res_w, int res_h) {
  const int width = img_w - 2, height = img_h - 2;
  const float halfWidth = (float)ceil((double)((float)res_w) / 2.0);
  const float halfHeight = (float)ceil((double)((float)res_h) / 2.0);
  const float xs[4] = {-halfWidth, -halfWidth, +halfWidth, +halfWidth};
  const float ys[4] = {-halfHeight, +halfHeight, -halfHeight, +halfHeight};
  bool touch = false;
#pragma unroll
  for (int i = 0; i < 4; i++) {
    float imx = ofsx + xs[i] * a11 + ys[i] * a12;
    float imy = ofsy + xs[i] * a21 + ys[i] * a22;
    if (floorf(imx) <= 0 || floorf(imy) <= 0 || ceilf(imx) >= width || ceilf(imy) >= height) touch = true;
  }
  return touch;
}

template <class T> __device__ __forceinline__ T *as_global(T *p) {
  typedef __attribute__((address_space(1))) T GT;
  GT *g = (GT *)(unsigned long long)p;
  return (T *)g;
}

__device__ __forceinline__ float lane_up1(float x) {
  return __int_as_float(__builtin_amdgcn_update_dpp(__float_as_int(x), __float_as_int(x), 0x138, 0xf, 0xf, false));
}
__device__ __forceinline__ float lane_down1(float x) {
  return __int_as_float(__builtin_amdgcn_update_dpp(__float_as_int(x), __float_as_int(x), 0x130, 0xf, 0xf, false));
}
__device__ __forceinline__ void wave_sync() {
  __builtin_amdgcn_fence(__ATOMIC_RELEASE, "wavefront");
  __builtin_amdgcn_wave_barrier();
  __builtin_amdgcn_fence(__ATOMIC_ACQUIRE, "wavefront");
}

__device__ __forceinline__ float fast_sqrtf(float x) {
  float s = __builtin_amdgcn_sqrtf(x);
  const float sd = __int_as_float(__float_as_int(s) - 1), su = __int_as_float(__float_as_int(s) + 1);
  const float vp = fmaf(-sd, s, x), vs = fmaf(-su, s, x);
  s = vp <= 0.f ? sd : s;
  s = vs > 0.f ? su : s;
  return s;
}
__device__ __forceinline__ float fast_sqrtf_any(float x) {
  const bool tiny = (unsigned)(__float_as_int(x) - 1) < (unsigned)(0x0f800000 - 1);
  if (__builtin_expect(__builtin_amdgcn_ballot_w64(tiny) != 0ull, 0)) return sqrtf(x);
  return fast_sqrtf(x);
}

struct __attribute__((packed, aligned(4))) PixPair { float a, b; };
struct __attribute__((packed, aligned(1))) PixPairU8 { unsigned char a, b; };
__device__ __forceinline__ void pix_pair(const float *__restrict__ p, float &a, float &b) { const PixPair q = *(const PixPair *)p; a = q.a; b = q.b; }
__device__ __forceinline__ void pix_pair(const unsigned char *__restrict__ p, float &a, float &b) {
  const PixPairU8 q = *(const PixPairU8 *)p;
  a = (float)q.a; b = (float)q.b;
}

struct TapLoads { float r00, r01, r10, r11, wx, wy; bool valid; };
template <class PX>
__device__ __forceinline__ TapLoads tap_load(const PX *__restrict__ im, int w, int h, float WX, float WY, bool touch) {
  TapLoads t;
  int x, y;
  if (!touch) { x = (int)WX; y = (int)WY; t.valid = true; }
  else { x = (int)floorf(WX); y = (int)floorf(WY); t.valid = WX >= 0 && WY >= 0 && x < w - 1 && y < h - 1; }
  t.wx = WX - (float)x;
  t.wy = WY - (float)y;
  if (t.valid) {
    const PX *Row0 = im + (size_t)y * w + x;
    pix_pair(Row0, t.r00, t.r01); pix_pair(Row0 + w, t.r10, t.r11);
  } else { t.r00 = t.r01 = t.r10 = t.r11 = 0.f; }
  return t;
}
template <class PX>
__device__ __forceinline__ TapLoads tap_load_bf(const PX *__restrict__ im, int w, int h, float WX, float WY, bool touch) {
  TapLoads t;
  const int x = (int)floorf(WX), y = (int)floorf(WY);
  t.valid = !touch || (WX >= 0 && WY >= 0 && x < w - 1 && y < h - 1);
  t.wx = WX - (float)x;
  t.wy = WY - (float)y;
  const int xc = min(max(x, 0), w - 2), yc = min(max(y, 0), h - 2);
  const PX *Row0 = im + (unsigned)(__mul24(yc, w) + xc);
  pix_pair(Row0, t.r00, t.r01); pix_pair(Row0 + w, t.r10, t.r11);
  return t;
}
__device__ __forceinline__ float tap_combine(const TapLoads &t) {
  if (!t.valid) return 0.f;
  const float I1 = t.wx * (t.r01 - t.r00) + t.r00;
  return t.wy * (t.wx * (t.r11 - t.r10) + t.r10 - I1) + I1;
}

template <class PX>
__device__ __forceinline__ TapLoads tap_load_inside(const PX *__restrict__ im, int w, float WX, float WY, bool inwin) {
  TapLoads t;
  const int x = (int)WX, y = (int)WY;
  t.valid = true;
  t.wx = WX - (float)x;
  t.wy = WY - (float)y;
  const PX *Row0 = im + (inwin ? (unsigned)(__mul24(y, w) + x) : 0u);
  pix_pair(Row0, t.r00, t.r01); pix_pair(Row0 + w, t.r10, t.r11);
  return t;
}
template <bool TOUCH, class PX>
__device__ __forceinline__ TapLoads tap_load_t(const PX *__restrict__ im, int w, int h, float WX, float WY, bool inwin) {
  if (TOUCH) return tap_load_bf(im, w, h, WX, WY, true);
  return tap_load_inside(im, w, WX, WY, inwin);
}
template <bool TOUCH> __device__ __forceinline__ float tap_combine_t(const TapLoads &t) {
  const float I1 = t.wx * (t.r01 - t.r00) + t.r00;
  const float v = t.wy * (t.wx * (t.r11 - t.r10) + t.r10 - I1) + I1;
  return (!TOUCH || t.valid) ? v : 0.f;
}

template <bool WIDE, bool TOUCH, class PX, class Store>
__device__ __forceinline__ void sample_tiles_rows_t(const PX *__restrict__ img, int w, int h, float fx, float fy, float a11, float a12,
                                                    float a21, float a22, int n, int row_begin, int row_end, int wv, int nw, Store store) {
  constexpr int TC = 8, TR = 64 / TC;
  const int half = n / 2;
  const int lane = threadIdx.x & 63, tcol = lane & (TC - 1), trow = lane / TC;
  float rx = fx - (float)half * a12;
  float ry = fy - (float)half * a22;
  for (int q = __builtin_amdgcn_readfirstlane(row_begin + wv * TR); q > 0; q--) { rx += a12; ry += a22; }
#pragma unroll
  for (int q = 0; q < TR - 1; q++) { const bool m = q < trow; const float nx = rx + a12, ny = ry + a22; rx = m ? nx : rx; ry = m ? ny : ry; }
  for (int r0 = row_begin + wv * TR; r0 < row_end; r0 += nw * TR) {
    const int row = r0 + trow;
    float WX = rx - (float)half * a11;
    float WY = ry - (float)half * a21;
#pragma unroll
    for (int q = 0; q < TC - 1; q++) { const bool m = q < tcol; const float nx = WX + a11, ny = WY + a21; WX = m ? nx : WX; WY = m ? ny : WY; }
    int c0 = 0;
    for (; WIDE && c0 + 8 * TC <= n; c0 += 8 * TC) {
      TapLoads t[8];
#pragma unroll
      for (int u = 0; u < 8; u++) {
        t[u] = tap_load_t<TOUCH>(img, w, h, WX, WY, row < row_end);
#pragma unroll
        for (int q = 0; q < TC; q++) { WX += a11; WY += a21; }
      }
#pragma unroll
      for (int u = 0; u < 8; u++)
        if (row < row_end) store(row, c0 + TC * u + tcol, tap_combine_t<TOUCH>(t[u]));
    }
    for (; c0 + 2 * TC < n; c0 += 4 * TC) {
      TapLoads t[4];
#pragma unroll
      for (int u = 0; u < 4; u++) {
        t[u] = tap_load_t<TOUCH>(img, w, h, WX, WY, row < row_end && c0 + TC * u + tcol < n);
#pragma unroll
        for (int q = 0; q < TC; q++) { WX += a11; WY += a21; }
      }
#pragma unroll
      for (int u = 0; u < 4; u++) {
        const int col = c0 + TC * u + tcol;
        if (row < row_end && col < n) store(row, col, tap_combine_t<TOUCH>(t[u]));
      }
    }
    for (; c0 < n; c0 += 2 * TC) {
      TapLoads t[2];
#pragma unroll
      for (int u = 0; u < 2; u++) {
        t[u] = tap_load_t<TOUCH>(img, w, h, WX, WY, row < row_end && c0 + TC * u + tcol < n);
#pragma unroll
        for (int q = 0; q < TC; q++) { WX += a11; WY += a21; }
      }
#pragma unroll
      for (int u = 0; u < 2; u++) {
        const int col = c0 + TC * u + tcol;
        if (row < row_end && col < n) store(row, col, tap_combine_t<TOUCH>(t[u]));
      }
    }
    if (r0 + nw * TR >= row_end) break;
    for (int q = nw * TR; q > 0; q--) { rx += a12; ry += a22; }
  }
}
template <bool WIDE, class PX, class Store>
__device__ __forceinline__ void sample_tiles_rows(const PX *__restrict__ img, int w, int h, float fx, float fy, float a11, float a12,
                                                  float a21, float a22, int n, int row_begin, int row_end, int wv, int nw, Store store) {
  const bool touch = __builtin_amdgcn_readfirstlane((int)check_borders(w, h, fx, fy, a11, a12, a21, a22, n, n)) != 0;
  if (touch) sample_tiles_rows_t<WIDE, true>(img, w, h, fx, fy, a11, a12, a21, a22, n, row_begin, row_end, wv, nw, store);
  else sample_tiles_rows_t<WIDE, false>(img, w, h, fx, fy, a11, a12, a21, a22, n, row_begin, row_end, wv, nw, store);
}
template <class PX, class Store>
// ... 60 lines not shown
```

mods-light-zmq_amd/csrc/pair.hip:

```cpp
#include "common.hpp"
#include "../../include/mods_degensac.h"
#include <algorithm>
#include <cmath>
#include <vector>

using namespace mods;

static bool dedup_on_device(const mods_pair_params *par) {
  return par->dup_before_ransac && par->dup_dist > 0 && par->dup_mode >= 0 && par->dup_mode <= 3;
}

static int ensure_tent2(mods_ctx *c) {
  MODS_HIP_CHECK(c->m_tent2.reserve(tent_bytes(((size_t)c->max_cand + 127) & ~(size_t)63) + 64));
  return MODS_OK;
}

static DupJob single_pair_dup_job(mods_ctx *c) {
  return {c->m_tent, c->m_tent2, c->m_count + count_slot(), c->m_count + kept_slot(), c->m_count + status_slot()};
}

constexpr size_t kPinArena = (size_t)24 << 20;

extern "C" __global__ __launch_bounds__(256) void u8_to_f32_kernel(const unsigned char *__restrict__ src, float *__restrict__ dst, size_t n4,
                                                                   size_t n) {
  for (size_t i = (size_t)blockIdx.x * 256 + threadIdx.x; i < n4; i += (size_t)gridDim.x * 256) {
    const uchar4 v = ((const uchar4 *)src)[i];
    ((float4 *)dst)[i] = make_float4((float)v.x, (float)v.y, (float)v.z, (float)v.w);
  }
  for (size_t i = 4 * n4 + (size_t)blockIdx.x * 256 + threadIdx.x; i < n; i += (size_t)gridDim.x * 256) dst[i] = (float)src[i];
}
extern "C" __global__ __launch_bounds__(256) void u8_rows_to_f32_kernel(const unsigned char *__restrict__ src, size_t stride, size_t w, size_t rows,
                                                                        float *__restrict__ dst) {
  for (size_t i = (size_t)blockIdx.x * 256 + threadIdx.x; i < rows * w; i += (size_t)gridDim.x * 256) dst[i] = (float)src[(i / w) * stride + i % w];
}
int mods::u8_stage_ensure(mods_ctx *c) {
  MODS_HIP_CHECK(c->u8_stage_dev.reserve((size_t)c->max_w * c->max_h * c->batch + 16));
  return MODS_OK;
}
int mods::u8_to_f32_launch(mods_ctx *c, const unsigned char *src, int n_img, int w, int h, int stride, float *dst) {
  const size_t n = (size_t)n_img * w * h;
  if (stride != w)
    hipLaunchKernelGGL(u8_rows_to_f32_kernel, dim3(1024), dim3(256), 0, c->stream, src, (size_t)stride, (size_t)w, (size_t)n_img * h, dst);
  else {
    const bool vec = (((uintptr_t)src & 3) | ((uintptr_t)dst & 15)) == 0;
    hipLaunchKernelGGL(u8_to_f32_kernel, dim3(1024), dim3(256), 0, c->stream, src, dst, vec ? n / 4 : (size_t)0, n);
  }
  MODS_HIP_CHECK(hipGetLastError());
  return MODS_OK;
}


int mods::pair_gpu_stage(mods_ctx *c, const float *img_dev, int w, int h, int stride, const mods_pair_params *par, mods_pair_result *res,
                         TentList *list) {
  if (!c || !img_dev || !par || !res || !list) { set_error("match_pair: null argument"); return MODS_E_ARG; }
  if (c->batch < 2) { set_error("match_pair needs a context created with batch >= 2"); return MODS_E_ARG; }
  memset(res, 0, sizeof(*res));
  for (int i = 0; i < 9; i++) res->H[i] = -1;
  int rc;
  const double t0 = now_ms();
  if ((rc = mods_detect_describe_dev(c, img_dev, 2, w, h, stride, &par->det, &par->desc, res->n_detected, res->n_described))) return rc;
  const double t1 = now_ms();
  res->ms_detect_describe = t1 - t0;
  if ((rc = match_run(c, c->regions_dev, res->n_described[0], c->regions_dev + c->max_cand, res->n_described[1],
                      par->fginn_ratio, par->contradDist, par->nn))) return rc;
  const bool dedup = dedup_on_device(par);
  if (dedup) {
    if ((rc = ensure_tent2(c))) return rc;
    const DupJob job = single_pair_dup_job(c);
    if ((rc = dup_filter_dev(c, &job, 1, res->n_described[0], par->dup_dist, par->dup_mode))) return rc;
  }
  MODS_HIP_CHECK(mods::stream_wait(c->stream));
  int n = read_slot(c->m_count, count_slot());
  res->n_tentatives = n;
  if (n > c->max_cand) { set_error("tentative list overflow"); return MODS_E_CAPACITY; }
  const bool filtered = dedup && read_slot(c->m_count, status_slot()) == 0;
  if (filtered) n = read_slot(c->m_count, kept_slot());
  list->resize(n);
  if (filtered) {
    res->n_unique = n;
    if (n > 0) {
      std::vector<char> stage(tent_bytes((size_t)n));
      MODS_HIP_CHECK(hipMemcpyAsync(stage.data(), c->m_tent2, stage.size(), hipMemcpyDeviceToHost, c->stream));
      MODS_HIP_CHECK(mods::stream_wait(c->stream));
      list->unpack_from(stage.data(), (size_t)n);
    }
  } else if ((rc = mods_match_copy_out(c, n, list->tent.data(), list->u6.data(), list->laf.data()))) return rc;
  res->ms_match = now_ms() - t1;
  return MODS_OK;
}

int mods::pairs_gpu_stage(mods_ctx *c, const void *const *img, const int *kinds, int n_pairs, int w, int h, const mods_pair_params *par,
                          mods_pair_result *const *res, TentList *const *lists) {
  if (!c || !img || !par || !res || !lists || n_pairs < 1) { set_error("match_pairs: null argument"); return MODS_E_ARG; }
  if (n_pairs == 1 && (!kinds || kinds[0] == 0) && !c->clahe_on) return pair_gpu_stage(c, (const float *)img[0], w, h, w, par, res[0], lists[0]);
  if (c->batch < 2 * n_pairs) { set_error("match_pairs: context batch %d < %d images", c->batch, 2 * n_pairs); return MODS_E_ARG; }
  if ((size_t)w * h > (size_t)c->max_w * c->max_h) { set_error("match_pairs: image larger than the context"); return MODS_E_ARG; }
  MODS_HIP_CHECK(hipSetDevice(c->device));
  const size_t plane2 = (size_t)2 * w * h;
  const int n_img = 2 * n_pairs;
  const bool clahe = c->clahe_on;
  bool all_u8 = !clahe && kinds != nullptr;
  for (int i = 0; all_u8 && i < n_pairs; i++) all_u8 = kinds[i] == 2;
  for (int i = 0; i < n_pairs; i++) {
    memset(res[i], 0, sizeof(*res[i]));
    for (int q = 0; q < 9; q++) res[i]->H[q] = -1;
    const int kind = kinds ? kinds[i] : 0;
    if (clahe && kind != 2) { set_error("match_pairs: a CLAHE pipeline takes 8-bit images only"); return MODS_E_ARG; }
    if (kind == 2) {
      if (int rc_stage = mods::u8_stage_ensure(c)) return rc_stage;
      unsigned char *st = c->u8_stage_dev + plane2 * i;
      if (!clahe && !all_u8 && ((plane2 & 3) || ((uintptr_t)st & 3))) { set_error("match_pairs: 8-bit input needs w*h*2 divisible by 4"); return MODS_E_ARG; }
      MODS_HIP_CHECK(hipMemcpyAsync(st, img[i], plane2, hipMemcpyHostToDevice, c->stream));
      const unsigned char *src = st;
      if (!clahe && !all_u8) hipLaunchKernelGGL(u8_to_f32_kernel, dim3(1024), dim3(256), 0, c->stream, src, c->input_dev + plane2 * i, plane2 / 4, plane2);
    } else {
      MODS_HIP_CHECK(hipMemcpyAsync(c->input_dev + plane2 * i, img[i], sizeof(float) * plane2,
                                    kind == 1 ? hipMemcpyHostToDevice : hipMemcpyDeviceToDevice, c->stream));
    }
  }
  MODS_HIP_CHECK(hipGetLastError());
  std::vector<int> nd(n_img), nr(n_img);
  int rc;
  if (clahe && (rc = clahe_launch(c, c->u8_stage_dev, n_img, w, h, w, &c->clahe_par, c->input_dev, w, 1))) return rc;
  const double t0 = now_ms();
  if (all_u8) rc = mods_detect_describe_dev_u8(c, c->u8_stage_dev, n_img, w, h, w, &par->det, &par->desc, nd.data(), nr.data());
  else rc = mods_detect_describe_dev(c, c->input_dev, n_img, w, h, w, &par->det, &par->desc, nd.data(), nr.data());
  if (rc) return rc;
  const double t1 = now_ms();
// ... 275 lines not shown
```

mods-light-zmq_amd/csrc/pipeline.hip:

```cpp
#include "common.hpp"
#include <condition_variable>
#include <deque>
#include <memory>
#include <mutex>
#include <thread>
#include <algorithm>
#include <chrono>
#include <time.h>
#include <pthread.h>
#include <sched.h>
#include <dirent.h>
#include <unistd.h>
#include <sys/syscall.h>
#include <map>
#include <set>
#include <tuple>

namespace mods {

struct Job {
  long tag = 0;
  const void *img = nullptr;
  int kind = 0;
  mods_pair_result res;
// ... 85 lines not shown
  wait_mode_for_worker(20000);
  worker_ready(p, mods_ransac_warmup(p->device, 16384));
  for (;;) {
    std::shared_ptr<Job> j;
    {
      std::unique_lock<std::mutex> lk(p->mu);
      p->cv_verify.wait(lk, [&] { return p->stop || !p->q_verify.empty(); });
      if (p->stop && p->q_verify.empty()) return;
      j = p->q_verify.front(); p->q_verify.pop_front();
    }
    if (j->rc == MODS_OK) {
      const long long c0 = thread_cpu_ns();
      j->rc = pair_verify_stage(p->device, &p->par, &j->res, &j->list, nullptr, 0, p->w, p->h);
      p->cpu_verify_ns.fetch_add(thread_cpu_ns() - c0, std::memory_order_relaxed);
      if (j->rc) j->err = mods_last_error();
    }
    {
      std::lock_guard<std::mutex> lk(p->mu);
      j->done = true;
    }
    p->cv_done.notify_all();
  }
}



extern "C" {

int mods_pipeline_create(int device, int w, int h, const mods_pair_params *par, int gpu_workers, int verify_workers,
                         mods_pipeline **out) {
  return mods_pipeline_create_ex(device, w, h, par, gpu_workers, verify_workers, 1, out);
}

int mods_pipeline_capacity(const mods_pipeline *p) { return p ? p->max_in_flight : 0; }

int mods_pipeline_timing_enable(mods_pipeline *p, int stage_mask) {
  if (!p) return MODS_E_ARG;
  for (auto *c : p->ctxs) { int rc = mods_ctx_timing_enable(c, stage_mask); if (rc) return rc; rc = mods_ctx_timing_reset(c); if (rc) return rc; }
  return MODS_OK;
}
int mods_pipeline_timing_read(mods_pipeline *p, int stage, double *total_ms, int *launches, double *bytes) {
  if (!p) return MODS_E_ARG;
  double ms = 0, by = 0; int n = 0;
  for (auto *c : p->ctxs) {
    double m1 = 0, b1 = 0; int n1 = 0;
    const int rc = mods_ctx_timing_read(c, stage, &m1, &n1, &b1);
    if (rc) return rc;
    ms += m1; by += b1; n += n1;
  }
  if (total_ms) *total_ms = ms;
  if (launches) *launches = n;
  if (bytes) *bytes = by;
  return MODS_OK;
}

long mods_pipeline_graph_replays(mods_pipeline *p) {
  long n = 0;
  if (p) for (auto *c : p->ctxs) n += mods_ctx_graph_replays(c);
  return n;
}
long mods_pipeline_u8_source_calls(mods_pipeline *p) {
  long n = 0;
  if (p) for (auto *c : p->ctxs) n += mods_ctx_u8_source_calls(c);
  return n;
}

int mods_pipeline_cpu_seconds(mods_pipeline *p, double *gpu_workers_s, double *verify_workers_s, int reset) {
  if (!p) return MODS_E_ARG;
  if (gpu_workers_s) *gpu_workers_s = p->cpu_gpu_ns.load() * 1e-9;
  if (verify_workers_s) *verify_workers_s = p->cpu_verify_ns.load() * 1e-9;
  if (reset) { p->cpu_gpu_ns.store(0); p->cpu_verify_ns.store(0); }
  return MODS_OK;
}

int mods_pipeline_match_mutual(mods_pipeline *p, int mode) {
  if (mode < 0 || mode > 2) { set_error("pipeline: match_mutual mode %d (0, 1 or 2)", mode); return MODS_E_ARG; }
  if (!p) { set_error("pipeline: null pipeline"); return MODS_E_ARG; }
  std::lock_guard<std::mutex> lk(p->mu);
  if (p->submitted) { set_error("pipeline: match_mutual after the first submit"); return MODS_E_ARG; }
  for (auto *c : p->ctxs) { const int rc = mods_ctx_match_mutual(c, mode); if (rc) return rc; }
  return MODS_OK;
}

int mods_pipeline_create_ex(int device, int w, int h, const mods_pair_params *par, int gpu_workers, int verify_workers,
                            int pairs_per_batch, mods_pipeline **out) {
  return mods_pipeline_create_clahe(device, w, h, par, gpu_workers, verify_workers, pairs_per_batch, nullptr, out);
}

int mods_pipeline_create_clahe(int device, int w, int h, const mods_pair_params *par, int gpu_workers, int verify_workers,
                               int pairs_per_batch, const mods_clahe_params *clahe, mods_pipeline **out) {
  if (!par || !out || gpu_workers < 1 || verify_workers < 1 || gpu_workers > 8 || verify_workers > 32 || pairs_per_batch < 1 ||
      pairs_per_batch > 16) { set_error("pipeline: bad arguments"); return MODS_E_ARG; }
  if (clahe && (clahe->tiles_x < 1 || clahe->tiles_x > 64 || clahe->tiles_y < 1 || clahe->tiles_y > 64 || w < 1 || h < 1)) {
    set_error("pipeline: CLAHE tile grid %d x %d outside [1, 64] or image %d x %d", clahe->tiles_x, clahe->tiles_y, w, h);
    return MODS_E_ARG;
  }
  std::unique_ptr<mods_pipeline> p(new mods_pipeline());
  p->device = device; p->w = w; p->h = h; p->par = *par;
  p->pairs_per_batch = pairs_per_batch;
  if (clahe) { p->clahe = true; p->clahe_par = *clahe; }
  p->max_in_flight = 2 * gpu_workers * pairs_per_batch + 2 * verify_workers;
  for (int i = 0; i < gpu_workers; i++) {
    mods_ctx *c = nullptr;
    int rc = mods_ctx_create_ex(device, w, h, 2 * pairs_per_batch, 1, &c);
    if (rc) { for (auto *q : p->ctxs) mods_ctx_destroy(q); return rc; }
    c->clahe_on = p->clahe; c->clahe_par = p->clahe_par;
    static const int streams_env = getenv("MODS_PIPELINE_STREAMS") ? atoi(getenv("MODS_PIPELINE_STREAMS")) : 1;
    if (streams_env >= 2) (void)mods_ctx_graphs(c, 1);
    else (void)mods_ctx_pyramid_streams(c, 1);
    p->ctxs.push_back(c);
  }
  for (int i = 0; i < gpu_workers; i++) p->gpu_threads.emplace_back(gpu_worker, p.get(), p->ctxs[i]);
  for (int i = 0; i < verify_workers; i++) p->verify_threads.emplace_back(verify_worker, p.get());
  {
    std::unique_lock<std::mutex> lk(p->mu);
    p->cv_ready.wait(lk, [&] { return p->ready == gpu_workers + verify_workers; });
  }
  if (p->warm_rc) {
    const int rc = p->warm_rc;
    const std::string err = p->warm_err;
    mods_pipeline_destroy(p.release());
    set_error("pipeline warm-up: %s", err.c_str());
    return rc;
  }
  *out = p.release();
  return MODS_OK;
}

static int submit_any(mods_pipeline *p, const void *img, int kind, long tag) {
  if (!p || !img) return MODS_E_ARG;
  auto j = std::make_shared<Job>();
  j->tag = tag; j->img = img; j->kind = kind;
  {
    std::unique_lock<std::mutex> lk(p->mu);
    p->cv_space.wait(lk, [&] { return (int)p->q_order.size() < p->max_in_flight; });
    p->submitted = true;
    p->q_gpu.push_back(j);
    p->q_order.push_back(j);
  }
  p->cv_gpu.notify_one();
  return MODS_OK;
}

static int refuse_f32(mods_pipeline *p) {
  if (p && p->clahe) { set_error("pipeline: CLAHE takes 8-bit images (mods_pipeline_submit_host_u8)"); return MODS_E_ARG; }
  return MODS_OK;
}
int mods_pipeline_submit(mods_pipeline *p, const float *img_dev, long tag) {
  if (const int rc = refuse_f32(p)) return rc;
  return submit_any(p, img_dev, 0, tag);
}
int mods_pipeline_submit_host(mods_pipeline *p, const float *img_host, long tag) {
  if (const int rc = refuse_f32(p)) return rc;
  return submit_any(p, img_host, 1, tag);
}
int mods_pipeline_submit_host_u8(mods_pipeline *p, const unsigned char *img_host, long tag) { return submit_any(p, img_host, 2, tag); }

int mods_pipeline_next_matches(mods_pipeline *p, mods_pair_result *res, long *tag, double *matches_out, int max_matches) {
  if (!p || !res) return MODS_E_ARG;
  std::shared_ptr<Job> j;
  {
    std::unique_lock<std::mutex> lk(p->mu);
    if (p->q_order.empty()) { set_error("pipeline: nothing in flight"); return MODS_E_ARG; }
    j = p->q_order.front();
    p->cv_done.wait(lk, [&] { return j->done; });
    p->q_order.pop_front();
// ... 26 lines not shown
```

mods-light-zmq_amd/csrc/sift.hip:

```cpp
#include "describe_common.hpp"
#include "detmath.hpp"
#include "device_util.hpp"

namespace mods {

constexpr int SMALL_CAP = 80;
#ifndef EXTRACT_T_LO
#define EXTRACT_T_LO 48
#endif
#ifndef EXTRACT_T_MID
#define EXTRACT_T_MID 64
#endif
#ifndef ES_MINB
#define ES_MINB 5
#endif

__device__ __forceinline__ double *lds_doubles(float *base, const void *p) {
  const int off = (int)((const float *)p - base);
  return (double *)(base + ((off + 1) & ~1));
}

struct RegionGeom {
  int P2;
  float scale;
// ... 442 lines not shown
    if (big) {
      const int li = s_w[wv][3] + p[3] - a[3], s0 = s_w[wv][4] + p[4] - a[4], r0 = s_w[wv][5] + p[5] - a[5], f0 = s_w[wv][6] + p[6] - a[6];
      const unsigned long long off = s_need[wv] + p_need - a_need;
      if (li >= max_regions || off + need > pool_elems || s0 + s_chunks > max_items || r0 + r_chunks * r_parts > max_items ||
          f0 + f_chunks > max_items || g.P2 >= 65536 || n_tap > k.tap_cap) {
        atomicExch(err_flag, 1);
      } else {
        BigRegion br;
        br.img = b; br.ri = ri; br.P2 = g.P2; br.n_tap = n_tap; br.slab = off; br.scale = g.scale; br.P2r = P2r;
        regions[li] = br;
        for (int c = 0; c < f_chunks; c++) fitems[f0 + c] = make_int2(li, c * f_rows);
        for (int c = 0; c < s_chunks; c++) sitems[s0 + c] = make_int2(li, c * BIG_SROWS);
        for (int c = 0; c < r_chunks; c++)
          for (int q = 0; q < r_parts; q++) ritems[r0 + c * r_parts + q] = make_int2(li, c * BIG_RROWS | (q * per << 16));
      }
    }
    __syncthreads();
  }
}

__global__ __launch_bounds__(256) void big_setup_kernel(DescConst k, const BigLists *__restrict__ bl, const BigRegion *__restrict__ regions,
                                                        int max_regions, float *__restrict__ pool, const int *__restrict__ err_flag) {
  extern __shared__ __attribute__((aligned(16))) float smem[];
  if (*err_flag) return;
  const int ps = k.desc_ps, ps2 = 2 * ps;
  float *s_tap = smem;
  float *s_seq = s_tap + k.tap_cap;
  int *s_cidx = (int *)(s_seq + ps2);
  double *s_red = lds_doubles(smem, s_cidx + ps2);
  const int n = min(bl->n_regions, max_regions);
  for (int li = blockIdx.x; li < n; li += gridDim.x) {
    const BigRegion br = regions[li];
    __syncthreads();
    blur_setup(br.P2, br.scale, ps, br.n_tap, s_tap, s_seq, s_cidx, s_red);
    float *hdr = pool + br.slab;
    for (int i = threadIdx.x; i < br.n_tap; i += 256) hdr[i] = s_tap[i];
    for (int i = threadIdx.x; i < ps; i += 256) hdr[br.n_tap + i] = s_seq[i];
    for (int i = threadIdx.x; i < ps2; i += 256) ((int *)(hdr + br.n_tap + ps))[i] = s_cidx[i];
  }
}

#define BIG_WAVE_LOOP(n_items, it) \
  for (int it = __builtin_amdgcn_readfirstlane((int)(blockIdx.x * 4 + (threadIdx.x >> 6))); it < (n_items); it += (int)gridDim.x * 4)

template <class PX>
__global__ __launch_bounds__(256) void big_sample_kernel(const PX *__restrict__ img_all, DescConst k, const BigLists *__restrict__ bl,
                                                         const BigRegion *__restrict__ regions, const int2 *__restrict__ sitems,
                                                         int max_items, const mods_region *__restrict__ reg_all,
                                                         float *__restrict__ pool, const int *__restrict__ err_flag) {
  if (*err_flag) return;
  const int n_items = min(bl->n_sitems, max_items);
  const int lane = threadIdx.x & 63;
  BIG_WAVE_LOOP(n_items, it) {
    const int2 item = sitems[it];
    const BigRegion br = regions[item.x];
    const RegionGeom g = region_geom(reg_all[(size_t)br.img * k.max_reg + br.ri], k.desc_mr, k.desc_ps, k.patch_rule);
    const PX *img = img_all + (size_t)k.w * k.h * br.img;
    const int P2 = br.P2, P2r = br.P2r, half = P2 / 2, w = k.w, h = k.h;
    const int row = item.y + 4 * (lane >> 4) + (lane & 3), s = (lane >> 2) & 3;
    if (row >= P2) continue;
    const bool touch = check_borders(w, h, g.fx, g.fy, g.f11, g.f12, g.f21, g.f22, P2, P2);
    float rx = g.fx - (float)half * g.f12;
    float ry = g.fy - (float)half * g.f22;
    for (int q = 0; q < row; q++) { rx += g.f12; ry += g.f22; }
    float WX = rx - (float)half * g.f11;
    float WY = ry - (float)half * g.f21;
    for (int q = 0; q < s; q++) { WX += g.f11; WY += g.f21; }
    float *dst = pool + br.slab + big_hdr_floats(br.n_tap, k.desc_ps) + (size_t)s * P2r + row;
    for (int c = s; c < P2; c += 32, dst += (size_t)32 * P2r) {
      float a0[8], b0[8], a1[8], b1[8];
      float wx[8], wy[8];
      bool ok[8];
#pragma unroll
      for (int u = 0; u < 8; u++) {
        ok[u] = false;
        if (c + 4 * u < P2) {
          int x, y;
          if (!touch) { x = (int)WX; y = (int)WY; ok[u] = true; }
          else { x = (int)floorf(WX); y = (int)floorf(WY); ok[u] = WX >= 0 && WY >= 0 && x < w - 1 && y < h - 1; }
          wx[u] = WX - (float)x;
          wy[u] = WY - (float)y;
          if (ok[u]) {
            const PX *Row0 = img + (size_t)y * w + x;
            pix_pair(Row0, a0[u], b0[u]);
            pix_pair(Row0 + w, a1[u], b1[u]);
          }
          WX += g.f11; WY += g.f21; WX += g.f11; WY += g.f21; WX += g.f11; WY += g.f21; WX += g.f11; WY += g.f21;
        }
      }
#pragma unroll
      for (int u = 0; u < 8; u++)
        if (c + 4 * u < P2) {
          float v = 0.f;
          if (ok[u]) {
            const float I1 = wx[u] * (b0[u] - a0[u]) + a0[u];
            v = wy[u] * (wx[u] * (b1[u] - a1[u]) + a1[u] - I1) + I1;
          }
          dst[(size_t)4 * u * P2r] = v;
        }
    }
  }
}

__global__ __launch_bounds__(256) void big_rowpass_kernel(DescConst k, const BigLists *__restrict__ bl, const BigRegion *__restrict__ regions,
                                                          const int2 *__restrict__ ritems, int max_items, float *__restrict__ pool,
                                                          const int *__restrict__ err_flag) {
  constexpr int TAPS_LDS = 1024;
  __shared__ float s_wtap[4][TAPS_LDS];
  if (*err_flag) return;
  const int ps = k.desc_ps, ps2 = t_stride(ps);
  const int n_items = min(bl->n_ritems, max_items);
  const int lane = threadIdx.x & 63;
  BIG_WAVE_LOOP(n_items, it) {
    const int2 item = ritems[it];
    const BigRegion br = regions[item.x];
    const int P2 = br.P2, P2r = br.P2r, n_tap = br.n_tap, r_tap = n_tap >> 1;
    const bool taps_in_lds = n_tap <= TAPS_LDS;
    wave_sync();
    if (taps_in_lds)
      for (int i = lane; i < n_tap; i += 64) s_wtap[threadIdx.x >> 6][i] = (pool + br.slab)[i];
    wave_sync();
    const int y = (item.y & 0xffff) + 4 * (lane & 15), pg = lane >> 4;
    const int step0 = item.y >> 16, step1 = min((ps + 3) / 4, step0 + big_rsteps(n_tap));
    const float *tap = taps_in_lds ? (const float *)s_wtap[threadIdx.x >> 6] : (const float *)(pool + br.slab);
    const int *cidx = (const int *)(pool + br.slab + n_tap + ps);
    const float *St = pool + br.slab + big_hdr_floats(n_tap, ps);
    float *T = (float *)St + big_s_floats(P2, P2r, n_tap);
    for (int step = step0; step < step1; step++) {
      const int pi = step * 4 + pg;
      const bool live = y < P2 && pi < ps;
      const int x0 = live ? cidx[2 * pi] : r_tap, x1 = live ? cidx[2 * pi + 1] : r_tap + 1;
      const bool interior = x0 - r_tap >= 0 && x0 + 1 + r_tap <= P2 - 1;
      const int yy = live ? y : 0;
      float4 s0, s1;
      if (__all(interior)) {
        const float *p = St + (size_t)(x0 - r_tap) * P2r + yy;
        float4 prev = *(const float4 *)p;
        float t = tap[0];
        s0 = make_float4(t * prev.x, t * prev.y, t * prev.z, t * prev.w);
        prev = *(const float4 *)(p + P2r);
        s1 = make_float4(t * prev.x, t * prev.y, t * prev.z, t * prev.w);
        int j = 1;
        for (; j + 7 < n_tap; j += 8) {
          float4 c[8];
#pragma unroll
          for (int u = 0; u < 8; u++) c[u] = *(const float4 *)(p + (size_t)(j + 1 + u) * P2r);
#pragma unroll
          for (int u = 0; u < 8; u++) {
            t = tap[j + u];
            s0.x = fmaf(t, prev.x, s0.x); s0.y = fmaf(t, prev.y, s0.y); s0.z = fmaf(t, prev.z, s0.z); s0.w = fmaf(t, prev.w, s0.w);
            s1.x = fmaf(t, c[u].x, s1.x); s1.y = fmaf(t, c[u].y, s1.y); s1.z = fmaf(t, c[u].z, s1.z); s1.w = fmaf(t, c[u].w, s1.w);
            prev = c[u];
          }
        }
        for (; j < n_tap; j++) {
          const float4 c = *(const float4 *)(p + (size_t)(j + 1) * P2r);
          t = tap[j];
          s0.x = fmaf(t, prev.x, s0.x); s0.y = fmaf(t, prev.y, s0.y); s0.z = fmaf(t, prev.z, s0.z); s0.w = fmaf(t, prev.w, s0.w);
          s1.x = fmaf(t, c.x, s1.x); s1.y = fmaf(t, c.y, s1.y); s1.z = fmaf(t, c.z, s1.z); s1.w = fmaf(t, c.w, s1.w);
          prev = c;
        }
      } else {
        const float *p = St + yy;
        int xa = x0 - r_tap; xa = xa < 0 ? 0 : (xa > P2 - 1 ? P2 - 1 : xa);
        float4 prev = *(const float4 *)(p + (size_t)xa * P2r);
        float t = tap[0];
        s0 = make_float4(t * prev.x, t * prev.y, t * prev.z, t * prev.w);
        xa = x0 - r_tap + 1; xa = xa < 0 ? 0 : (xa > P2 - 1 ? P2 - 1 : xa);
// ... 648 lines not shown
      }
      wave_sync();
      bool changed = false;
      {
        const int rr = lane >> 3;
        if ((redo >> (8 * rr)) & 1) {
          const double inv = tmp[rr];
          for (int i = lane & 7; i < 128; i += 8) {
            double *vp = acc + s2_vec(rr, i);
            double x = *vp * inv;
            if (pass == 0 && x > k.max_bin) { x = k.max_bin; changed = true; }
            *vp = x;
          }
        }
      }
      const unsigned long long ch = __ballot(changed);
      unsigned long long next = 0;
      for (int rr = 0; rr < SW_R; rr++)
        if ((ch >> (8 * rr)) & 0xffull) next |= 0xffull << (8 * rr);
      redo = next;
      wave_sync();
      if (!redo) break;
    }
    if (k.root) {
      if (lane < SW_R) {
        double sum = 0.;
#pragma unroll 1
        for (int i = 0; i < 128; i += 8) {
          double x[8];
#pragma unroll
          for (int q = 0; q < 8; q++) x[q] = acc[s2_vec(lane, i + q)];
#pragma unroll
          for (int q = 0; q < 8; q++) sum += fabs(x[q]);
        }
        tmp[lane] = sum;
      }
      wave_sync();
    }
    {
      const int rr = lane >> 3;
      if (ri0 + rr < n) {
        const double rs = k.root ? tmp[rr] : 1.0;
        uint32_t *out = (uint32_t *)reg[ri0 + rr].desc;
        for (int w4 = lane & 7; w4 < 32; w4 += 8) {
          uint32_t word = 0;
#pragma unroll
          for (int q = 0; q < 4; q++) {
            const double x = acc[s2_vec(rr, 4 * w4 + q)];
            const double y = k.root ? sqrt(x / rs) : x;
            int bq = (int)(512.0 * y + 0.5);
            bq = bq < 255 ? bq : 255;
            bq = bq > 0 ? bq : 0;
            word |= (uint32_t)bq << (8 * q);
          }
          out[w4] = word;
        }
      }
    }
    S2PROF(5)
#ifdef SIFT_PROF
    pn++;
#endif
  }
#ifdef SIFT_PROF
  if (lane == 0 && (blockIdx.x % 64) == 3 && wv == 1)
    printf("sift_wave2 prof: block %d units %d cycles per unit: other %llu photo %llu grad %llu hist %llu shift+norm %llu norms %llu\n", blockIdx.x, pn,
           pt[0] / max(pn, 1), pt[1] / max(pn, 1), pt[2] / max(pn, 1), pt[3] / max(pn, 1), pt[4] / max(pn, 1), pt[5] / max(pn, 1));
#endif
}

__global__ __launch_bounds__(256) void sift_patch_test_kernel(const float *__restrict__ patch, int ps, int root, double max_bin,
                                                              const float *__restrict__ mask, const SiftTab *__restrict__ tab,
                                                              uint8_t *out) {
  extern __shared__ __attribute__((aligned(16))) float smem[];
  SiftLds L(smem, ps);
  sift_tables(tab, ps, L.w);
  for (int i = threadIdx.x; i < 256; i += 256) L.lut[i] = g_atan_lut[i];
  for (int p = threadIdx.x; p < ps * ps; p += 256) L.patch[p] = patch[p];
  __syncthreads();
  sift_from_patch(L.patch, mask, L.w, L.lut, ps, root != 0, max_bin, L.px, L.bo, L.vec, L.red, out);
}

int launch_extract_and_sift(mods_ctx *ctx, const float *img_dev, int n_img, DescConst k, const float *dmask, const SiftTab *tab, bool run_sift,
                            const unsigned char *img_u8) {
  StageScope ts(ctx, MODS_STAGE_DESCRIBE);
  const int ps = k.desc_ps, ps2 = 2 * ps, pp = ps * ps;
  const size_t patch_elems = (size_t)n_img * k.reg_cap * pp;
  const int max_big = 1 << 17, max_items = 1 << 20;
  const int small_cap_items = n_img * k.reg_cap;
  const size_t book_elems = (sizeof(BigLists) + sizeof(BigRegion) * max_big + 3 * sizeof(int2) * max_items + 3 * sizeof(int) * (size_t)small_cap_items + 15) / 4;
  const unsigned long long area_units = std::max<unsigned long long>(1, ((unsigned long long)k.w * k.h + (1ull << 21) - 1) >> 21);
  const unsigned long long pool_elems = std::max<unsigned long long>(256ull << 20, (unsigned long long)n_img * area_units * (64ull << 20));
  const size_t need = patch_elems + book_elems + pool_elems;
  MODS_HIP_CHECK(mods::reserve_pool(ctx, ctx->desc_scratch, need, need));
  float *patches = ctx->desc_scratch;
  BigLists *bl = (BigLists *)(ctx->desc_scratch + patch_elems);
  BigRegion *bregs = (BigRegion *)(bl + 1);
  int2 *sitems = (int2 *)(bregs + max_big);
  int2 *ritems = sitems + max_items;
  int2 *fitems = ritems + max_items;
  int *small_items = (int *)(fitems + max_items);
  float *pool = ctx->desc_scratch + patch_elems + book_elems;
  MODS_HIP_CHECK(hipMemsetAsync(bl, 0, sizeof(BigLists), ctx->stream));
  { const int trc = launch_blur_table(ctx, ps); if (trc) return trc; }
  {
  StageScope ts_extract(ctx, MODS_STAGE_EXTRACT);
  k.tap_cap = 4096;
  const int small_cap = SMALL_CAP;
  k.p2_hi = small_cap;
  hipLaunchKernelGGL(big_classify_kernel, dim3(CLASSIFY_BLOCKS, n_img), dim3(1024), 0, ctx->stream, k, ctx->regions_dev,
                     ctx->region_count, bl, bregs, sitems, ritems, fitems, small_items, small_cap_items, std::min(small_cap, EXTRACT_T_LO), std::min(small_cap, EXTRACT_T_MID), max_big, max_items,
                     pool_elems, ctx->desc_err_dev);
  {
    const int tiers[4] = {-1, std::min(small_cap, EXTRACT_T_LO), std::min(small_cap, EXTRACT_T_MID), small_cap};
    for (int t = 0; t < 3; t++) {
      if (tiers[t + 1] <= tiers[t]) continue;
      DescConst kt = k;
      kt.p2_lo = tiers[t]; kt.p2_hi = tiers[t + 1];
      const size_t capS = kt.p2_hi > 4 ? kt.p2_hi : 4;
      const size_t ldsS = sizeof(float) * (capS * odd4((int)capS) + capS * ((capS + 3) & ~(size_t)3) + 2 * ps2 + 32) + 32;
      if (img_u8 && kernel_from_u8(ctx, U8K_EXTRACT_SMALL))
        hipLaunchKernelGGL(extract_small_kernel<unsigned char>, dim3(4096), dim3(256), ldsS, ctx->stream, img_u8, kt, ctx->regions_dev,
                           small_items + (size_t)t * small_cap_items, &bl->n_small[t], small_cap_items, patches,
                           (const float *)ctx->blur_table_dev);
      else
        hipLaunchKernelGGL(extract_small_kernel<float>, dim3(4096), dim3(256), ldsS, ctx->stream, img_dev, kt, ctx->regions_dev,
                           small_items + (size_t)t * small_cap_items, &bl->n_small[t], small_cap_items, patches,
                           (const float *)ctx->blur_table_dev);
    }
  }
  const size_t ldsH = sizeof(float) * (k.tap_cap + 4 * ps2) + 32;
  hipLaunchKernelGGL(big_setup_kernel, dim3(1024), dim3(256), ldsH, ctx->stream, k, bl, bregs, max_big, pool, ctx->desc_err_dev);
  if (img_u8 && kernel_from_u8(ctx, U8K_BIG_FUSED))
    hipLaunchKernelGGL(big_fused_kernel<unsigned char>, dim3(8192), dim3(256), BIG_FUSE_KB * 1024, ctx->stream, img_u8, k, bl, bregs, fitems,
                       max_items, ctx->regions_dev, pool, ctx->desc_err_dev);
  else
    hipLaunchKernelGGL(big_fused_kernel<float>, dim3(8192), dim3(256), BIG_FUSE_KB * 1024, ctx->stream, img_dev, k, bl, bregs, fitems,
                       max_items, ctx->regions_dev, pool, ctx->desc_err_dev);
  if (img_u8 && kernel_from_u8(ctx, U8K_BIG_SAMPLE))
    hipLaunchKernelGGL(big_sample_kernel<unsigned char>, dim3(4096), dim3(256), 0, ctx->stream, img_u8, k, bl, bregs, sitems, max_items,
                       ctx->regions_dev, pool, ctx->desc_err_dev);
  else
    hipLaunchKernelGGL(big_sample_kernel<float>, dim3(4096), dim3(256), 0, ctx->stream, img_dev, k, bl, bregs, sitems, max_items,
                       ctx->regions_dev, pool, ctx->desc_err_dev);
  hipLaunchKernelGGL(big_rowpass_kernel, dim3(4096), dim3(256), 0, ctx->stream, k, bl, bregs, ritems, max_items, pool,
                     ctx->desc_err_dev);
  hipLaunchKernelGGL(big_colres_kernel, dim3(4096), dim3(256), 0, ctx->stream, k, bl, bregs, max_big, pool, patches, ctx->desc_err_dev);
  }
  StageScope ts_sift(ctx, MODS_STAGE_SIFT);
  if (run_sift && ps > 45)
    hipLaunchKernelGGL(sift_kernel, dim3(2048, n_img), dim3(256), sift_lds_bytes(ps), ctx->stream, k, patches, ctx->regions_dev,
                       ctx->region_count, dmask, tab);
  else if (run_sift) {
    static DynLdsOnce once16, once18;
    MODS_HIP_CHECK(dyn_lds_once(once16, (const void *)sift_wave2_kernel<16>, 160 * 1024, ctx->device));
    MODS_HIP_CHECK(dyn_lds_once(once18, (const void *)sift_wave2_kernel<SW_CW>, 160 * 1024, ctx->device));
    int span = 0;
    {
      const float step = 5.0f / (float)(2 * (ps >> 1));
      for (int bc = 0; bc < 4; bc++) {
        int lo = ps, hi = -1;
        for (int i = 0; i < ps; i++) {
          const float x = step * i; const int xi = (int)x; const float w1 = x - xi, w0 = 1.0f - w1;
          const bool on = (xi - 1 == bc && w0 > 0) || (xi == bc && w1 > 0);
          if (on) { lo = std::min(lo, i); hi = i; }
        }
        if (hi >= lo) span = std::max(span, hi - lo + 1);
      }
    }
    for (int b0 = 0; b0 < n_img; b0 += S2_MAX_IMG) {
      const int nb = std::min(S2_MAX_IMG, n_img - b0);
      if (b0) MODS_HIP_CHECK(hipMemsetAsync(&bl->sift_next, 0, sizeof(int), ctx->stream));
      const float *pch = patches + (size_t)b0 * k.reg_cap * pp;
      mods_region *regs = ctx->regions_dev + (size_t)b0 * k.max_reg;
      if (span <= 16)
        hipLaunchKernelGGL(sift_wave2_kernel<16>, dim3(ctx->n_cu), dim3(64 * S2_WAVES), sift_wave2_lds_bytes(ps), ctx->stream, k, pch,
                           regs, ctx->region_count + b0, dmask, tab, nb, &bl->sift_next);
      else
        hipLaunchKernelGGL(sift_wave2_kernel<SW_CW>, dim3(ctx->n_cu), dim3(64 * S2_WAVES), sift_wave2_lds_bytes(ps), ctx->stream, k, pch,
                           regs, ctx->region_count + b0, dmask, tab, nb, &bl->sift_next);
    }
  }
  MODS_HIP_CHECK(hipGetLastError());
  return MODS_OK;
}

int launch_half_sift(mods_ctx *ctx, int n_img, DescConst k, const float *dmask, const SiftTab *tab) {
  StageScope ts(ctx, MODS_STAGE_DESCRIBE);
  MODS_HIP_CHECK(ctx->regions_half_dev.reserve((size_t)ctx->max_cand * ctx->batch));
  MODS_HIP_CHECK(hipMemcpyAsync(ctx->regions_half_dev, ctx->regions_dev, sizeof(mods_region) * (size_t)ctx->max_cand * n_img,
                                hipMemcpyDeviceToDevice, ctx->stream));
  k.half_desc = 1;
  const int ps = k.desc_ps;
  const float *patches = ctx->desc_scratch;
  hipLaunchKernelGGL(sift_kernel, dim3(2048, n_img), dim3(256), sift_lds_bytes(ps), ctx->stream, k, patches, ctx->regions_half_dev,
                     ctx->region_count, dmask, tab);
  MODS_HIP_CHECK(hipGetLastError());
  return MODS_OK;
}

int launch_sift_patch_test(mods_ctx *ctx, const float *patch_dev, int ps, int root, double max_bin, uint8_t *out_dev) {
  hipLaunchKernelGGL(sift_patch_test_kernel, dim3(1), dim3(256), sift_lds_bytes(ps), ctx->stream, patch_dev, ps, root, max_bin,
                     ctx->desc_tables_dev + kTabDescMask, (const SiftTab *)(ctx->desc_tables_dev + kTabSift), out_dev);
  MODS_HIP_CHECK(hipGetLastError());
  return MODS_OK;
}

}
```

Baseline: 1039.

## Add interleaved pair-row u8 twin image for bilinear tap gathers

The u8-to-f32 conversion now also writes a twin image where each pixel is stored next to the pixel below it. Orient, small extract and big fused kernels read this layout by default, so each bilinear tap becomes one 4-byte load instead of two 2-byte loads from different rows. The cost is an extra 2-bytes-per-pixel buffer written during conversion and more template instantiations. A test entry point and a pipeline mask setter are added to control and check the path.

```diff
diff --git a/include/mods_hip.h b/include/mods_hip.h
--- a/include/mods_hip.h
+++ b/include/mods_hip.h
@@ -96,6 +96,8 @@
 long mods_ctx_graph_replays(const mods_ctx *ctx);
 long mods_ctx_u8_source_calls(const mods_ctx *ctx);
 int mods_ctx_u8_kernels(mods_ctx *ctx, int mask);
+int mods_ctx_pair_rows_test(mods_ctx *ctx, const unsigned char *batch, int n_img, int w, int h, int src_offset, float *f32_out,
+                            unsigned char *pairs_out);
 int mods_ctx_pyramid_streams(mods_ctx *ctx, int n);
 int mods_ctx_timing_read(mods_ctx *ctx, int stage, double *total_ms, int *launches, double *bytes);
 int mods_ctx_timing_reset(mods_ctx *ctx);
@@ -404,6 +406,7 @@
 int mods_pipeline_timing_enable(mods_pipeline *p, int stage_mask);
 int mods_pipeline_timing_read(mods_pipeline *p, int stage, double *total_ms, int *launches, double *bytes);
 long mods_pipeline_u8_source_calls(mods_pipeline *p);
+int mods_pipeline_u8_kernels(mods_pipeline *p, int mask);
 long mods_pipeline_graph_replays(mods_pipeline *p);
 int mods_pipeline_cpu_seconds(mods_pipeline *p, double *gpu_workers_s, double *verify_workers_s, int reset);
 int mods_pipeline_submit(mods_pipeline *p, const float *img_dev, long tag);
diff --git a/mods-light-zmq_amd/__init__.py b/mods-light-zmq_amd/__init__.py
--- a/mods-light-zmq_amd/__init__.py
+++ b/mods-light-zmq_amd/__init__.py
@@ -401,6 +401,15 @@
 
     def set_u8_kernels(self, mask):
         _check(lib().mods_ctx_u8_kernels(self.h, int(mask)))
+
+    def pair_rows_test(self, batch_u8, src_offset=0):
+        a = np.ascontiguousarray(batch_u8, np.uint8)
+        n, h, w = a.shape
+        f32 = np.zeros((n, h, w), np.float32)
+        raw = np.zeros(2 * a.size + 16, np.uint8)
+        _check(lib().mods_ctx_pair_rows_test(self.h, C.c_void_p(a.ctypes.data), n, w, h, int(src_offset), C.c_void_p(f32.ctypes.data),
+                                             C.c_void_p(raw.ctypes.data)))
+        return f32, raw[:2 * a.size].reshape(n, h, w, 2), raw[2 * a.size:]
 
     def set_match_mutual(self, mode):
         _check(lib().mods_ctx_match_mutual(self.h, int(mode)))
@@ -1172,6 +1181,9 @@
     def set_match_mutual(self, mode):
         _check(lib().mods_pipeline_match_mutual(self.h, int(mode)))
 
+    def set_u8_kernels(self, mask):
+        _check(lib().mods_pipeline_u8_kernels(self.h, int(mask)))
+
     def submit(self, dev_ptr, tag=0):
         _check(lib().mods_pipeline_submit(self.h, C.c_void_p(dev_ptr), C.c_long(tag)))
 
diff --git a/mods-light-zmq_amd/csrc/capi.hip b/mods-light-zmq_amd/csrc/capi.hip
--- a/mods-light-zmq_amd/csrc/capi.hip
+++ b/mods-light-zmq_amd/csrc/capi.hip
@@ -407,7 +407,7 @@
   const bool can = c->dd_graphs && c->timing_mask == 0 && !mods::has_hooks(c) && !mods::has_nets(c) && det->detectorType != MODS_DET_MSER;
   if (!can) { mods::dev_state_changed(c); return dd_enqueue(c, img_dev, n_img, w, h, stride, det, desc); }
   mods_ctx::DdKey key;
-  key.img = img_dev; key.img_u8 = c->img_u8_dev; key.n_img = n_img; key.w = w; key.h = h; key.stride = stride;
+  key.img = img_dev; key.img_u8 = c->img_u8_dev; key.img_pairs = c->img_pairs_dev; key.n_img = n_img; key.w = w; key.h = h; key.stride = stride;
   key.par_hash = fnv1a(desc, sizeof(*desc), fnv1a(det, sizeof(*det), 1469598103934665603ull)) ^ (unsigned long long)c->pyr_streams;
   key.epoch = c->dev_state_epoch;
   if (c->dd_stale) { dd_graph_drop(c); c->dd_linear.clear(); c->dd_stale = false; }
@@ -464,9 +464,28 @@
 long mods_ctx_graph_replays(const mods_ctx *c) { return c ? c->dd_replays : 0; }
 long mods_ctx_u8_source_calls(const mods_ctx *c) { return c ? c->u8_source_calls : 0; }
 int mods_ctx_u8_kernels(mods_ctx *c, int mask) {
-  if (!c || mask > 15) { set_error("u8_kernels: bad argument"); return MODS_E_ARG; }
+  if (!c || mask > 255) { set_error("u8_kernels: bad argument"); return MODS_E_ARG; }
   c->u8_kernels = mask < 0 ? -1 : mask;
   mods::dev_state_changed(c);
+  return MODS_OK;
+}
+
+int mods_ctx_pair_rows_test(mods_ctx *c, const unsigned char *batch, int n_img, int w, int h, int src_offset, float *f32_out,
+                            unsigned char *pairs_out) {
+  if (!c || !batch || !f32_out || !pairs_out) { set_error("pair_rows_test: null argument"); return MODS_E_ARG; }
+  if (n_img < 1 || n_img > c->batch || w < 1 || h < 1 || (size_t)w * h > (size_t)c->max_w * c->max_h || src_offset < 0 || src_offset > 15) {
+    set_error("pair_rows_test: bad argument"); return MODS_E_ARG;
+  }
+  MODS_HIP_CHECK(hipSetDevice(c->device));
+  int rc;
+  unsigned char *pairs = nullptr;
+  if ((rc = mods::u8_stage_ensure(c)) || (rc = mods::pairs_ensure(c, &pairs, true))) return rc;
+  const size_t n = (size_t)n_img * w * h;
+  MODS_HIP_CHECK(hipMemsetAsync(pairs, 0xee, 2 * n + 16, c->stream));
+  MODS_HIP_CHECK(hipMemcpyAsync(c->u8_stage_dev + src_offset, batch, n, hipMemcpyHostToDevice, c->stream));
+  if ((rc = mods::u8_to_f32_launch(c, c->u8_stage_dev + src_offset, n_img, w, h, w, c->input_dev, pairs))) return rc;
+  MODS_HIP_CHECK(hipMemcpyAsync(f32_out, c->input_dev, sizeof(float) * n, hipMemcpyDeviceToHost, c->stream));
+  MODS_HIP_CHECK(mods::copy_wait(c->stream, pairs_out, pairs, 2 * n + 16, hipMemcpyDeviceToHost));
   return MODS_OK;
 }
 
@@ -500,7 +519,7 @@
   if (n_img < 1 || n_img > c->batch) { set_error("detect_describe: %d images, context batch %d", n_img, c->batch); return MODS_E_ARG; }
   if (stride < w) { set_error("detect_describe: stride %d < width %d", stride, w); return MODS_E_ARG; }
   MODS_HIP_CHECK(hipSetDevice(c->device));
-  c->img_u8_dev = nullptr;
+  c->img_u8_dev = c->img_pairs_dev = nullptr;
   return dd_call(c, img_dev, n_img, w, h, stride, det, desc, n_detected_host, n_regions_host);
 }
 
@@ -513,11 +532,15 @@
   if (stride < w) { set_error("detect_describe_u8: stride %d < width %d", stride, w); return MODS_E_ARG; }
   MODS_HIP_CHECK(hipSetDevice(c->device));
   int rc;
-  if ((rc = mods::u8_to_f32_launch(c, img_u8_dev, n_img, w, h, stride, c->input_dev))) return rc;
-  c->img_u8_dev = (stride == w && det->detectorType != MODS_DET_MSER) ? img_u8_dev : nullptr;
+  const bool twin = stride == w && det->detectorType != MODS_DET_MSER;
+  unsigned char *pairs = nullptr;
+  if (twin && (rc = mods::pairs_ensure(c, &pairs))) return rc;
+  if ((rc = mods::u8_to_f32_launch(c, img_u8_dev, n_img, w, h, stride, c->input_dev, pairs))) return rc;
+  c->img_u8_dev = twin ? img_u8_dev : nullptr;
+  c->img_pairs_dev = pairs;
   if (c->img_u8_dev) c->u8_source_calls++;
   rc = dd_call(c, c->input_dev, n_img, w, h, w, det, desc, n_detected_host, n_regions_host);
-  c->img_u8_dev = nullptr;
+  c->img_u8_dev = c->img_pairs_dev = nullptr;
   return rc;
 }
 
@@ -652,11 +675,14 @@
   MODS_HIP_CHECK(hipMemcpyAsync(c->keys_dev, keys, sizeof(mods_affkey) * n_keys, hipMemcpyHostToDevice, c->stream));
   MODS_HIP_CHECK(hipMemcpyAsync(c->cand_count + 2 * c->batch, &n_keys, sizeof(int), hipMemcpyHostToDevice, c->stream));
   MODS_HIP_CHECK(mods::stream_wait(c->stream));
-  if ((rc = mods::u8_to_f32_launch(c, c->u8_stage_dev, 1, w, h, w, c->input_dev))) return rc;
+  unsigned char *pairs = nullptr;
+  if ((rc = mods::pairs_ensure(c, &pairs))) return rc;
+  if ((rc = mods::u8_to_f32_launch(c, c->u8_stage_dev, 1, w, h, w, c->input_dev, pairs))) return rc;
   c->img_u8_dev = c->u8_stage_dev;
+  c->img_pairs_dev = pairs;
   c->u8_source_calls++;
   rc = describe_run(c, c->input_dev, 1, w, h, par);
-  c->img_u8_dev = nullptr;
+  c->img_u8_dev = c->img_pairs_dev = nullptr;
   if (rc) return rc;
   if ((rc = mods_regions_fetch(c, 0, out, max_out, n_out))) return rc;
   return check_desc_err(c);
diff --git a/mods-light-zmq_amd/csrc/common.hpp b/mods-light-zmq_amd/csrc/common.hpp
--- a/mods-light-zmq_amd/csrc/common.hpp
+++ b/mods-light-zmq_amd/csrc/common.hpp
@@ -193,6 +193,8 @@
   mods::PinnedBuf<int> host_counts;
   mods::Buf<unsigned char> u8_stage_dev;
   const unsigned char *img_u8_dev = nullptr;
+  mods::Buf<unsigned char> pair_rows_dev;
+  const unsigned char *img_pairs_dev = nullptr;
   int u8_kernels = -1;
   long u8_source_calls = 0;
   mods::Buf<unsigned char> clahe_lut;
@@ -272,8 +274,9 @@
   int timing_mask = 0;
   bool dd_graphs = false;
   struct DdKey { const float *img = nullptr; const unsigned char *img_u8 = nullptr;
+                 const unsigned char *img_pairs = nullptr;
                  int n_img = 0, w = 0, h = 0, stride = 0; unsigned long long par_hash = 0, epoch = ~0ull;
-                 bool operator==(const DdKey &o) const { return img == o.img && img_u8 == o.img_u8 && n_img == o.n_img && w == o.w && h == o.h && stride == o.stride && par_hash == o.par_hash && epoch == o.epoch; } };
+                 bool operator==(const DdKey &o) const { return img == o.img && img_u8 == o.img_u8 && img_pairs == o.img_pairs && n_img == o.n_img && w == o.w && h == o.h && stride == o.stride && par_hash == o.par_hash && epoch == o.epoch; } };
   unsigned long long dev_state_epoch = 0;
   std::vector<std::pair<DdKey, hipGraphExec_t>> dd_cache;
   bool dd_stale = false;
@@ -348,7 +351,8 @@
 int ransac_profile_mode();
 
 int describe_run(mods_ctx *ctx, const float *img_dev, int n_img, int w, int h, const mods_describe_params *par);
-int u8_to_f32_launch(mods_ctx *c, const unsigned char *src, int n_img, int w, int h, int stride, float *dst);
+int u8_to_f32_launch(mods_ctx *c, const unsigned char *src, int n_img, int w, int h, int stride, float *dst, unsigned char *pairs = nullptr);
+int pairs_ensure(mods_ctx *c, unsigned char **pairs, bool always = false);
 int u8_stage_ensure(mods_ctx *c);
 int describe_run_view(mods_ctx *ctx, const float *img_dev, int n_img, int w, int h, const mods_describe_params *par, const double *H,
                       int orig_w, int orig_h, mods_region *det_copy_dev);
diff --git a/mods-light-zmq_amd/csrc/describe.hip b/mods-light-zmq_amd/csrc/describe.hip
--- a/mods-light-zmq_amd/csrc/describe.hip
+++ b/mods-light-zmq_amd/csrc/describe.hip
@@ -718,6 +718,7 @@
   const bool external = ctx->ext_fn != nullptr || ctx->ext_net != nullptr;
   const bool hooks = external || ctx->shape_fn || ctx->shape_net || ctx->ori_fn || ctx->ori_net;
   const unsigned char *img_u8 = (!H && !hooks) ? ctx->img_u8_dev : nullptr;
+  const unsigned char *img_pairs = img_u8 ? ctx->img_pairs_dev : nullptr;
   if (external && par->fastExtraction) { set_error("FastPatchExtraction with an external descriptor is not supported"); return MODS_E_ARG; }
   if (external) { k.desc_mr = ctx->ext_mr; k.desc_ps = ctx->ext_ps; k.photo = 0; k.patch_rule = 1; }
   int *key_count = ctx->cand_count + 2 * ctx->batch;
@@ -734,7 +735,10 @@
       const size_t need = sizeof(OriOut) * (size_t)k.ori_cap * ctx->max_cand * ctx->batch;
       MODS_HIP_CHECK(mods::reserve_pool(ctx, ctx->ori_multi_dev, need, need));
     }
-    if (img_u8 && kernel_from_u8(ctx, U8K_ORIENT))
+    if (img_pairs && kernel_from_pairs(ctx, U8K_ORIENT))
+      hipLaunchKernelGGL(orient_kernel<PairPx>, dim3(8192, n_img), dim3(64), lds, ctx->stream, (const PairPx *)img_pairs, k, ctx->keys_dev,
+                         key_count, orimask, (OriOut *)ctx->ori_dev.get(), (OriOut *)ctx->ori_multi_dev.get());
+    else if (img_u8 && kernel_from_u8(ctx, U8K_ORIENT))
       hipLaunchKernelGGL(orient_kernel<unsigned char>, dim3(8192, n_img), dim3(64), lds, ctx->stream, img_u8, k, ctx->keys_dev, key_count,
                          orimask, (OriOut *)ctx->ori_dev.get(), (OriOut *)ctx->ori_multi_dev.get());
     else
@@ -748,7 +752,7 @@
                          (const OriOut *)ctx->ori_dev.get(), ctx->regions_dev, ctx->region_count, ctx->inside_count);
     MODS_HIP_CHECK(hipGetLastError());
   }
-  rc = launch_extract_and_sift(ctx, img_dev, n_img, k, dmask, tab, !external, img_u8);
+  rc = launch_extract_and_sift(ctx, img_dev, n_img, k, dmask, tab, !external, img_u8, img_pairs);
   if (rc) return rc;
   ctx->have_half = false;
   if (par->halfDesc && !external) {
diff --git a/mods-light-zmq_amd/csrc/describe_common.hpp b/mods-light-zmq_amd/csrc/describe_common.hpp
--- a/mods-light-zmq_amd/csrc/describe_common.hpp
+++ b/mods-light-zmq_amd/csrc/describe_common.hpp
@@ -46,13 +46,30 @@
 #ifndef BIG_SAMPLE_FROM_U8
 #define BIG_SAMPLE_FROM_U8 0
 #endif
-enum { U8K_ORIENT = 1, U8K_EXTRACT_SMALL = 2, U8K_BIG_FUSED = 4, U8K_BIG_SAMPLE = 8 };
+#ifndef ORIENT_FROM_PAIRS
+#define ORIENT_FROM_PAIRS 1
+#endif
+#ifndef EXTRACT_SMALL_FROM_PAIRS
+#define EXTRACT_SMALL_FROM_PAIRS 1
+#endif
+#ifndef BIG_FUSED_FROM_PAIRS
+#define BIG_FUSED_FROM_PAIRS 1
+#endif
+#ifndef BIG_SAMPLE_FROM_PAIRS
+#define BIG_SAMPLE_FROM_PAIRS 0
+#endif
+enum { U8K_ORIENT = 1, U8K_EXTRACT_SMALL = 2, U8K_BIG_FUSED = 4, U8K_BIG_SAMPLE = 8, U8K_PAIRS_SHIFT = 4 };
 constexpr int kU8KernelsDefault = (ORIENT_FROM_U8 ? U8K_ORIENT : 0) | (EXTRACT_SMALL_FROM_U8 ? U8K_EXTRACT_SMALL : 0) |
-                                  (BIG_FUSED_FROM_U8 ? U8K_BIG_FUSED : 0) | (BIG_SAMPLE_FROM_U8 ? U8K_BIG_SAMPLE : 0);
-inline bool kernel_from_u8(const mods_ctx *ctx, int kernel) { return ((ctx->u8_kernels < 0 ? kU8KernelsDefault : ctx->u8_kernels) & kernel) != 0; }
+                                  (BIG_FUSED_FROM_U8 ? U8K_BIG_FUSED : 0) | (BIG_SAMPLE_FROM_U8 ? U8K_BIG_SAMPLE : 0) |
+                                  ((ORIENT_FROM_PAIRS ? U8K_ORIENT : 0) | (EXTRACT_SMALL_FROM_PAIRS ? U8K_EXTRACT_SMALL : 0) |
+                                   (BIG_FUSED_FROM_PAIRS ? U8K_BIG_FUSED : 0) | (BIG_SAMPLE_FROM_PAIRS ? U8K_BIG_SAMPLE : 0)) << U8K_PAIRS_SHIFT;
+inline int u8_kernels_mask(const mods_ctx *ctx) { return ctx->u8_kernels < 0 ? kU8KernelsDefault : ctx->u8_kernels; }
+inline bool kernel_from_pairs(const mods_ctx *ctx, int kernel) { return (u8_kernels_mask(ctx) & (kernel << U8K_PAIRS_SHIFT)) != 0; }
+inline bool kernel_from_u8(const mods_ctx *ctx, int kernel) { return (u8_kernels_mask(ctx) & kernel) != 0 && !kernel_from_pairs(ctx, kernel); }
+inline bool any_kernel_from_pairs(const mods_ctx *ctx) { return (u8_kernels_mask(ctx) >> U8K_PAIRS_SHIFT) != 0; }
 
 int launch_extract_and_sift(mods_ctx *ctx, const float *img_dev, int n_img, DescConst k, const float *dmask, const SiftTab *tab,
-                            bool run_sift = true, const unsigned char *img_u8 = nullptr);
+                            bool run_sift = true, const unsigned char *img_u8 = nullptr, const unsigned char *img_pairs = nullptr);
 int launch_half_sift(mods_ctx *ctx, int n_img, DescConst k, const float *dmask, const SiftTab *tab);
 int launch_sift_patch_test(mods_ctx *ctx, const float *patch_dev, int ps, int root, double max_bin, uint8_t *out_dev);
 
diff --git a/mods-light-zmq_amd/csrc/device_util.hpp b/mods-light-zmq_amd/csrc/device_util.hpp
--- a/mods-light-zmq_amd/csrc/device_util.hpp
+++ b/mods-light-zmq_amd/csrc/device_util.hpp
@@ -59,6 +59,16 @@
 __device__ __forceinline__ void pix_pair(const unsigned char *__restrict__ p, float &a, float &b) {
   const PixPairU8 q = *(const PixPairU8 *)p;
   a = (float)q.a; b = (float)q.b;
+}
+struct __attribute__((packed, aligned(2))) PairPx { unsigned char p, below; };
+struct __attribute__((packed, aligned(2))) TapQuadU8 { unsigned char r00, r10, r01, r11; };
+template <class PX>
+__device__ __forceinline__ void tap_pixels(const PX *__restrict__ Row0, int w, float &r00, float &r01, float &r10, float &r11) {
+  pix_pair(Row0, r00, r01); pix_pair(Row0 + w, r10, r11);
+}
+__device__ __forceinline__ void tap_pixels(const PairPx *__restrict__ Row0, int, float &r00, float &r01, float &r10, float &r11) {
+  const TapQuadU8 q = *(const TapQuadU8 *)Row0;
+  r00 = (float)q.r00; r01 = (float)q.r01; r10 = (float)q.r10; r11 = (float)q.r11;
 }
 
 struct TapLoads { float r00, r01, r10, r11, wx, wy; bool valid; };
@@ -72,7 +82,7 @@
   t.wy = WY - (float)y;
   if (t.valid) {
     const PX *Row0 = im + (size_t)y * w + x;
-    pix_pair(Row0, t.r00, t.r01); pix_pair(Row0 + w, t.r10, t.r11);
+    tap_pixels(Row0, w, t.r00, t.r01, t.r10, t.r11);
   } else { t.r00 = t.r01 = t.r10 = t.r11 = 0.f; }
   return t;
 }
@@ -85,7 +95,7 @@
   t.wy = WY - (float)y;
   const int xc = min(max(x, 0), w - 2), yc = min(max(y, 0), h - 2);
   const PX *Row0 = im + (unsigned)(__mul24(yc, w) + xc);
-  pix_pair(Row0, t.r00, t.r01); pix_pair(Row0 + w, t.r10, t.r11);
+  tap_pixels(Row0, w, t.r00, t.r01, t.r10, t.r11);
   return t;
 }
 __device__ __forceinline__ float tap_combine(const TapLoads &t) {
@@ -102,7 +112,7 @@
   t.wx = WX - (float)x;
   t.wy = WY - (float)y;
   const PX *Row0 = im + (inwin ? (unsigned)(__mul24(y, w) + x) : 0u);
-  pix_pair(Row0, t.r00, t.r01); pix_pair(Row0 + w, t.r10, t.r11);
+  tap_pixels(Row0, w, t.r00, t.r01, t.r10, t.r11);
   return t;
 }
 template <bool TOUCH, class PX>
diff --git a/mods-light-zmq_amd/csrc/pair.hip b/mods-light-zmq_amd/csrc/pair.hip
--- a/mods-light-zmq_amd/csrc/pair.hip
+++ b/mods-light-zmq_amd/csrc/pair.hip
@@ -1,4 +1,5 @@
 #include "common.hpp"
+#include "describe_common.hpp"
 #include "../../include/mods_degensac.h"
 #include <algorithm>
 #include <cmath>
@@ -33,17 +34,45 @@
                                                                         float *__restrict__ dst) {
   for (size_t i = (size_t)blockIdx.x * 256 + threadIdx.x; i < rows * w; i += (size_t)gridDim.x * 256) dst[i] = (float)src[(i / w) * stride + i % w];
 }
+extern "C" __global__ __launch_bounds__(256) void u8_to_f32_pairs_kernel(const unsigned char *__restrict__ src, float *__restrict__ dst,
+                                                                         unsigned char *__restrict__ pairs, size_t n4, size_t n, size_t w, size_t h) {
+  for (size_t i = (size_t)blockIdx.x * 256 + threadIdx.x; i < n4; i += (size_t)gridDim.x * 256) {
+    const bool last = (4 * i / w) % h == h - 1;
+    const uchar4 v = ((const uchar4 *)src)[i];
+    const uchar4 b = last ? v : *(const uchar4 *)(src + 4 * i + w);
+    ((float4 *)dst)[i] = make_float4((float)v.x, (float)v.y, (float)v.z, (float)v.w);
+    ((uint2 *)pairs)[i] = make_uint2((unsigned)v.x | (unsigned)b.x << 8 | (unsigned)v.y << 16 | (unsigned)b.y << 24,
+                                     (unsigned)v.z | (unsigned)b.z << 8 | (unsigned)v.w << 16 | (unsigned)b.w << 24);
+  }
+  for (size_t i = 4 * n4 + (size_t)blockIdx.x * 256 + threadIdx.x; i < n; i += (size_t)gridDim.x * 256) {
+    const unsigned char v = src[i], b = (i / w) % h == h - 1 ? v : src[i + w];
+    dst[i] = (float)v;
+    ((unsigned short *)pairs)[i] = (unsigned short)(v | b << 8);
+  }
+}
 int mods::u8_stage_ensure(mods_ctx *c) {
   MODS_HIP_CHECK(c->u8_stage_dev.reserve((size_t)c->max_w * c->max_h * c->batch + 16));
   return MODS_OK;
 }
-int mods::u8_to_f32_launch(mods_ctx *c, const unsigned char *src, int n_img, int w, int h, int stride, float *dst) {
+int mods::pairs_ensure(mods_ctx *c, unsigned char **pairs, bool always) {
+  *pairs = nullptr;
+  if (!always && !any_kernel_from_pairs(c)) return MODS_OK;
+  const size_t need = (size_t)2 * c->max_w * c->max_h * c->batch + 16;
+  MODS_HIP_CHECK(mods::reserve_pool(c, c->pair_rows_dev, need, need));
+  *pairs = c->pair_rows_dev;
+  return MODS_OK;
+}
+int mods::u8_to_f32_launch(mods_ctx *c, const unsigned char *src, int n_img, int w, int h, int stride, float *dst, unsigned char *pairs) {
   const size_t n = (size_t)n_img * w * h;
-  if (stride != w)
+  if (stride != w) {
+    if (pairs) { set_error("u8_to_f32: the pair-row twin needs packed rows"); return MODS_E_ARG; }
     hipLaunchKernelGGL(u8_rows_to_f32_kernel, dim3(1024), dim3(256), 0, c->stream, src, (size_t)stride, (size_t)w, (size_t)n_img * h, dst);
-  else {
+  } else {
     const bool vec = (((uintptr_t)src & 3) | ((uintptr_t)dst & 15)) == 0;
-    hipLaunchKernelGGL(u8_to_f32_kernel, dim3(1024), dim3(256), 0, c->stream, src, dst, vec ? n / 4 : (size_t)0, n);
+    if (pairs) {
+      const bool vec4 = vec && (w & 3) == 0 && ((uintptr_t)pairs & 7) == 0;
+      hipLaunchKernelGGL(u8_to_f32_pairs_kernel, dim3(1024), dim3(256), 0, c->stream, src, dst, pairs, vec4 ? n / 4 : (size_t)0, n, (size_t)w, (size_t)h);
+    } else hipLaunchKernelGGL(u8_to_f32_kernel, dim3(1024), dim3(256), 0, c->stream, src, dst, vec ? n / 4 : (size_t)0, n);
   }
   MODS_HIP_CHECK(hipGetLastError());
   return MODS_OK;
diff --git a/mods-light-zmq_amd/csrc/pipeline.hip b/mods-light-zmq_amd/csrc/pipeline.hip
--- a/mods-light-zmq_amd/csrc/pipeline.hip
+++ b/mods-light-zmq_amd/csrc/pipeline.hip
@@ -191,6 +191,14 @@
   return MODS_OK;
 }
 
+int mods_pipeline_u8_kernels(mods_pipeline *p, int mask) {
+  if (!p) { set_error("pipeline: null pipeline"); return MODS_E_ARG; }
+  std::lock_guard<std::mutex> lk(p->mu);
+  if (p->submitted) { set_error("pipeline: u8_kernels after the first submit"); return MODS_E_ARG; }
+  for (auto *c : p->ctxs) { const int rc = mods_ctx_u8_kernels(c, mask); if (rc) return rc; }
+  return MODS_OK;
+}
+
 int mods_pipeline_create_ex(int device, int w, int h, const mods_pair_params *par, int gpu_workers, int verify_workers,
                             int pairs_per_batch, mods_pipeline **out) {
   return mods_pipeline_create_clahe(device, w, h, par, gpu_workers, verify_workers, pairs_per_batch, nullptr, out);
diff --git a/mods-light-zmq_amd/csrc/sift.hip b/mods-light-zmq_amd/csrc/sift.hip
--- a/mods-light-zmq_amd/csrc/sift.hip
+++ b/mods-light-zmq_amd/csrc/sift.hip
@@ -548,8 +548,7 @@
           wy[u] = WY - (float)y;
           if (ok[u]) {
             const PX *Row0 = img + (size_t)y * w + x;
-            pix_pair(Row0, a0[u], b0[u]);
-            pix_pair(Row0 + w, a1[u], b1[u]);
+            tap_pixels(Row0, w, a0[u], b0[u], a1[u], b1[u]);
           }
           WX += g.f11; WY += g.f21; WX += g.f11; WY += g.f21; WX += g.f11; WY += g.f21; WX += g.f11; WY += g.f21;
         }
@@ -1364,7 +1363,8 @@
 }
 
 int launch_extract_and_sift(mods_ctx *ctx, const float *img_dev, int n_img, DescConst k, const float *dmask, const SiftTab *tab, bool run_sift,
-                            const unsigned char *img_u8) {
+                            const unsigned char *img_u8, const unsigned char *img_pairs) {
+  const PairPx *img_pr = (const PairPx *)img_pairs;
   StageScope ts(ctx, MODS_STAGE_DESCRIBE);
   const int ps = k.desc_ps, ps2 = 2 * ps, pp = ps * ps;
   const size_t patch_elems = (size_t)n_img * k.reg_cap * pp;
@@ -1401,7 +1401,11 @@
       kt.p2_lo = tiers[t]; kt.p2_hi = tiers[t + 1];
       const size_t capS = kt.p2_hi > 4 ? kt.p2_hi : 4;
       const size_t ldsS = sizeof(float) * (capS * odd4((int)capS) + capS * ((capS + 3) & ~(size_t)3) + 2 * ps2 + 32) + 32;
-      if (img_u8 && kernel_from_u8(ctx, U8K_EXTRACT_SMALL))
+      if (img_pr && kernel_from_pairs(ctx, U8K_EXTRACT_SMALL))
+        hipLaunchKernelGGL(extract_small_kernel<PairPx>, dim3(4096), dim3(256), ldsS, ctx->stream, img_pr, kt, ctx->regions_dev,
+                           small_items + (size_t)t * small_cap_items, &bl->n_small[t], small_cap_items, patches,
+                           (const float *)ctx->blur_table_dev);
+      else if (img_u8 && kernel_from_u8(ctx, U8K_EXTRACT_SMALL))
         hipLaunchKernelGGL(extract_small_kernel<unsigned char>, dim3(4096), dim3(256), ldsS, ctx->stream, img_u8, kt, ctx->regions_dev,
                            small_items + (size_t)t * small_cap_items, &bl->n_small[t], small_cap_items, patches,
                            (const float *)ctx->blur_table_dev);
@@ -1413,13 +1417,19 @@
   }
   const size_t ldsH = sizeof(float) * (k.tap_cap + 4 * ps2) + 32;
   hipLaunchKernelGGL(big_setup_kernel, dim3(1024), dim3(256), ldsH, ctx->stream, k, bl, bregs, max_big, pool, ctx->desc_err_dev);
-  if (img_u8 && kernel_from_u8(ctx, U8K_BIG_FUSED))
+  if (img_pr && kernel_from_pairs(ctx, U8K_BIG_FUSED))
+    hipLaunchKernelGGL(big_fused_kernel<PairPx>, dim3(8192), dim3(256), BIG_FUSE_KB * 1024, ctx->stream, img_pr, k, bl, bregs, fitems,
+                       max_items, ctx->regions_dev, pool, ctx->desc_err_dev);
+  else if (img_u8 && kernel_from_u8(ctx, U8K_BIG_FUSED))
     hipLaunchKernelGGL(big_fused_kernel<unsigned char>, dim3(8192), dim3(256), BIG_FUSE_KB * 1024, ctx->stream, img_u8, k, bl, bregs, fitems,
                        max_items, ctx->regions_dev, pool, ctx->desc_err_dev);
   else
     hipLaunchKernelGGL(big_fused_kernel<float>, dim3(8192), dim3(256), BIG_FUSE_KB * 1024, ctx->stream, img_dev, k, bl, bregs, fitems,
                        max_items, ctx->regions_dev, pool, ctx->desc_err_dev);
-  if (img_u8 && kernel_from_u8(ctx, U8K_BIG_SAMPLE))
+  if (img_pr && kernel_from_pairs(ctx, U8K_BIG_SAMPLE))
+    hipLaunchKernelGGL(big_sample_kernel<PairPx>, dim3(4096), dim3(256), 0, ctx->stream, img_pr, k, bl, bregs, sitems, max_items,
+                       ctx->regions_dev, pool, ctx->desc_err_dev);
+  else if (img_u8 && kernel_from_u8(ctx, U8K_BIG_SAMPLE))
     hipLaunchKernelGGL(big_sample_kernel<unsigned char>, dim3(4096), dim3(256), 0, ctx->stream, img_u8, k, bl, bregs, sitems, max_items,
                        ctx->regions_dev, pool, ctx->desc_err_dev);
   else
```

New measurement: 1057 (median of 6 runs). About the same (+1.8%).
